# Chris10M/Lip2Speech

Hardware: AMD Instinct MI355X
Metric: mel-frames/sec at LRW batch=32, 29-frame clips (Lip2Speech.inference, S=300) (higher is better)
Workload: dtype f32; 1 GPU; LRW single-word, batch=32 per step, 29x96x96 RGB mouth crops, S=300 decode steps, speaker embedding supplied (encoding=voice), random-init weights; every step is one full pass over one B=32 batch; frames=29, decode_steps=300, library=libl2s_hip.so, parallelism=dp1 (clip sharding, no collective), batches_per_launch_chain=8, launch_chains_in_flight_per_gpu=3, distinct_batches_per_gpu=24, ranks=1

## Files before the change

### include/l2s_diag.h

```cpp
#ifndef L2S_DIAG_H
#define L2S_DIAG_H

#include "l2s.h"

#ifdef __cplusplus
extern "C" {
#endif


int l2s_op_gemm(const float* A, const float* Wt, const float* scale, const float* shift, const float* actw,
                float* C, int M, int N, int K, int act, void* stream);
int l2s_op_conv1d(const float* X, const float* Wp, const float* scale, const float* shift, const float* actw,
                  float* out, int B, int Tin, int Cin, int Cout, int taps, int stride, int pad, int act,
                  void* stream);
int l2s_op_gemm_ex(const float* A, const float* Wt, const float* scale, const float* shift, const float* actw, float* C, int M, int N,
                   int K, int act, int flags, void* stream);
int l2s_op_conv1d_ex(const float* X, const float* Wp, const float* scale, const float* shift, const float* actw, float* out, int B,
                     int Tin, int Cin, int Cout, int taps, int stride, int pad, int act, int flags, void* stream);
int l2s_op_conv1d_bwd(const float* dZ, const float* X, const float* Wp, float* dX, float* dWp, int B, int Tin, int Cin, int Cout, int taps,
                      int stride, int pad, void* stream);
int l2s_op_frontend(l2s_model* m, const float* video, int B, int T, int H, int W, float* out, void* stream);
int l2s_op_face_conv2d(const float* x, int64_t x_bstride, int B, int H, int W, int Cin, const float* w, const float* scale, const float* shift,
                       const float* res, int relu, float* y, int Cout, int kh, int kw, int stride, int ph, int pw, void* stream);
int l2s_op_face_taps(l2s_model* m, const float* faces, int64_t batch_stride, int B, float* const* taps, float* proj, float* emb, void* ws,
                     int64_t ws_bytes, void* stream);
int l2s_op_speaker_taps(l2s_model* m, const float* audio, int B, int n_samples, float* const* taps, float* emb, void* ws, int64_t ws_bytes, void* stream);
int l2s_op_speaker_taps_packed(l2s_model* m, const float* audio_packed, const int64_t* offsets, const int64_t* n_samples, int B, float* const* taps, float* emb,
                               void* ws, int64_t ws_bytes, void* stream);
int l2s_op_encoder_taps(l2s_model* m, const float* video, int B, int T, int H, int W, float* const* taps, float* feat, void* ws, int64_t ws_bytes,
                        void* stream);
int l2s_op_lstm_cell_chain(l2s_model* m, int B, int n_pairs, void* ws, int64_t ws_bytes, void* stream, double* avg_us);
int l2s_op_launch_chain(int kind, int n_launches, int blocks, int n_per_block, const float* in, float* out, void* stream);
int l2s_op_skinny_timeline(void* ts_dev);
int l2s_op_attn_timeline(void* ts_dev);
int l2s_op_flat_timeline(void* ts_dev);
int l2s_op_pdecode_timeline(void* ts_dev, int step);
int l2s_op_gemm_x3_timeline(void* ts_dev, int block);
int l2s_op_fused_unit_timeline(void* ts_dev, int h);
int l2s_op_step_attn_chain(l2s_model* m, float* state, int B, int T, int n_launches, void* ws, int64_t ws_bytes, void* stream);
int l2s_op_launch_chain2(int kind, int n_launches, int blocks, int n_per_block, const float* in, float* out, void* stream_a, void* stream_b);
int l2s_op_stamp_log(void* log_dev, int64_t capacity);

#ifdef __cplusplus
}
#endif
#endif
```

### lip2speech_amd/csrc/l2s_api.hip

```cpp
#include "../../include/l2s.h"
#ifdef L2S_DIAG
#include "../../include/l2s_diag.h"
#endif
#include "l2s_common.h"
#include "l2s_model.h"
#include "pdecode.h"

#include <algorithm>
#include <cmath>
#include <functional>
#include <cstring>
#include <map>
#include <memory>
#include <mutex>
#include <string>
#include <unordered_map>
#include <vector>

namespace l2s {

static thread_local std::string g_err;
void set_error(const std::string& msg) { g_err = msg; }

static Options g_default_opt;
// ... 56 lines not shown
void prof_count(const char* name, int64_t n) {
    if (!g_prof_on) return;
    std::lock_guard<std::mutex> lk(g_prof_mu);
    auto it = g_prof_idx.find(name);
    if (it == g_prof_idx.end()) {
        g_prof_idx[name] = (int)g_prof.size();
        g_prof.push_back(ProfEntry{name});
        it = g_prof_idx.find(name);
    }
    g_prof[it->second].launches += n;
}
static void prof_drain() {
    std::lock_guard<std::mutex> lk(g_prof_mu);
    for (auto& e : g_prof) {
        for (auto& pr : e.pending) {
            (void)hipEventSynchronize(pr.second);
            float ms = 0.f;
            if (hipEventElapsedTime(&ms, pr.first, pr.second) == hipSuccess) e.total_ms += ms;
            (void)hipEventDestroy(pr.first);
            (void)hipEventDestroy(pr.second);
        }
        e.pending.clear();
    }
}

}

namespace l2s {

struct EncPlan {
    int NF, Hp;
    int64_t act_a, act_b, t1, t2, last;
};
static EncPlan enc_plan(int NF, int H) {
    EncPlan p{};
    p.NF = NF;
    p.Hp = H / 4;
    int64_t hw = (int64_t)p.Hp * p.Hp;
    int64_t amax = (int64_t)p.NF * hw * STAGE_CH[0], t1 = 0, t2 = 0;
    int cin = STAGE_CH[0];
    int h = p.Hp;
    for (int st = 0; st < 3; ++st) {
        int cout = STAGE_CH[st + 1], half = cout / 2;
        int ho = (h + 1) / 2;
        int64_t in_px = (int64_t)p.NF * h * h, out_px = (int64_t)p.NF * ho * ho;
        t1 = std::max(t1, std::max(in_px * half, out_px * half));
        t2 = std::max(t2, std::max(out_px * cin, out_px * half));
        amax = std::max(amax, out_px * cout);
        cin = cout;
        h = ho;
    }
    p.act_a = amax; p.act_b = amax; p.t1 = t1; p.t2 = t2;
    p.last = (int64_t)p.NF * h * h * LAST_CH;
    return p;
}
static int64_t enc_ws_floats(int NF, int H) {
    EncPlan p = enc_plan(NF, H);
    return p.act_a + p.act_b + p.t1 + p.t2 + p.last + 64 * 8;
}

static int64_t prologue_ws_floats(int B, int T) {
    int L[4];
    int m = content_lens(T, L);
    int64_t BT = (int64_t)B * T, n = 0;
    n += BT * 4096;
    n += BT * 1024;
    n += BT * 512;
    n += (int64_t)B * 512 * 2;
    n += (int64_t)pad16(B) * 512 * 6;
    n += (int64_t)B * 1024;
    n += BT * 4608;
    for (int j = 0; j < 4; ++j) n += (int64_t)B * L[j] * 512;
    n += (int64_t)B * m * 2560;
    n += (int64_t)B * m * 256 * 4;
    n += (int64_t)B * m * (VOC + VOCP);
    n += 8 * std::max((int64_t)B * m * 256, (int64_t)B * 512);
    for (int j = 1; j < 4; ++j) n += (int64_t)CT_KS[j] * B * L[j] * 512;
    n += 8 * BT * 512;
    if (B <= 2) n += pbilstm_ws_bytes() / 4 + 64;
    return n + 64 * 44;
}
static int64_t decode_ws_floats(int B) {
    int64_t Bp = pad16(B);
    return Bp * (512 * 4 + 512 * 2 + 512 + 256 * 4 + 96) + (int64_t)B * (512 + 256 + 256) + 64 * 24 + (B + 2 + 64)  + (B <= 8 ? pdecode_ws_bytes(B) / 4 + 64 : 0);
}
constexpr int POST_TAPSPLIT_ROWS = 640;
static int64_t postnet_ws_floats(int B, int S) { return (int64_t)B * S * 512 * ((int64_t)B * S <= POST_TAPSPLIT_ROWS * MAX_GROUP ? 9 : 4) + 64 * 7; }


static GemmP pw_gemm(const float* A, int lda, int a_off, const ConvW& c, float* C, int ldc, int c_off, int cstride,
                     int64_t M, int N, int K, int act) {
    GemmP p = gemm_plain(A + a_off, lda, c.W, C + c_off, ldc, (int)M, N, K);
    p.scale = c.scale; p.shift = c.shift; p.actw = c.actw; p.act = act; p.c_cstride = cstride;
    p.W3 = c.W3;
    return p;
}

static FrameSrc frame_src(const float* video, int B) { FrameSrc f{}; f.p[0] = video; f.per = B; return f; }

#define S1_RUN_CHAINED(m, U, run, h) \
    ((m)->opt.trunk_chain && ((h) >= 6 || (m)->opt.trunk_chain >= 2) && (m)->opt.trunk_x3 && (U).pw1_p3 && (U).pw2_p3 && (run) >= 2 && (run) <= S1_CHAIN_MAX)
#ifdef L2S_DIAG
static int enc_tap(float* const* taps, int i, const float* src, int64_t n, hipStream_t s) {
    if (taps && taps[i]) L2S_CHECK_HIP(hipMemcpyAsync(taps[i], src, (size_t)n * sizeof(float), hipMemcpyDeviceToDevice, s));
    return 0;
}
static int enc_tap_interior(int u) {
    set_error("l2s: encoder tap of unit " + std::to_string(u) + " asked for, but the unit is interior to a stage-chain launch and its output never reaches memory (option \"trunk_chain\")");
    return 1;
}
static int enc_taps_check(const l2s_model* m, float* const* taps, int h) {
    if (!taps || !m->opt.fuse_trunk) return 0;
    for (int u = 0; u < N_UNITS; ++u) {
        const UnitW& U = m->w.unit[u];
        if (U.stride2) { h = (h + 1) / 2; continue; }
        int run = 1;
        while (u + run < N_UNITS && !m->w.unit[u + run].stride2 && m->w.unit[u + run].half == U.half) ++run;
        if (!S1_RUN_CHAINED(m, U, run, h)) continue;
        for (int i = 0; i < run - 1; ++i)
            if (taps[1 + u + i]) return enc_tap_interior(u + i);
        u += run - 1;
    }
    return 0;
}
#define L2S_ENC_TAP(i, src, n) do { if (enc_tap(taps, i, src, n, s)) return 1; } while (0)
#define L2S_ENC_TAPS_ARG , float* const* taps = nullptr
#else
#define L2S_ENC_TAP(i, src, n) do {} while (0)
#define L2S_ENC_TAPS_ARG
#endif
static int encoder_run(l2s_model* m, const FrameSrc& video, int B, int T, int H, int W, const float* emb, float* vis,
                       float* feat, void* ws, int64_t ws_bytes, hipStream_t s, const RaggedTab* rg = nullptr L2S_ENC_TAPS_ARG) {
    X3Scope x3scope(m->opt.infer_bf16 ? 0 : m->opt.gemm_x3);
    Bf16Scope bf16scope(m->opt.infer_bf16);
    const Weights& w = m->w;
    EncPlan pl = enc_plan(rg ? rg->NF : B * T, H);
    Bump bp(ws, ws_bytes);
    float* a = bp.f(pl.act_a); float* b = bp.f(pl.act_b); float* t1 = bp.f(pl.t1); float* t2 = bp.f(pl.t2); float* last = bp.f(pl.last);
    L2S_REQUIRE(!bp.overflow, "encoder workspace too small");
#ifdef L2S_DIAG
    if (enc_taps_check(m, taps, pl.Hp)) return 1;
#endif
    FrontendW fe = w.fe;
    if (!m->opt.frontend_x3) fe.w3 = nullptr;
    fe.pair = m->opt.frontend_x3 >= 2; fe.pipe = m->opt.frontend_x3 == 3;
    fe.solo = m->opt.frontend_solo && (m->opt.frontend_solo >= 2 || chains_hint() >= 2);
    if (!m->opt.infer_bf16) fe.w1 = nullptr;
    if (rg ? launch_frontend_ragged(fe, video, *rg, H, W, a, s) : launch_frontend(fe, video, B, T, H, W, a, s)) return 1;
    L2S_ENC_TAP(0, a, (int64_t)pl.NF * pl.Hp * pl.Hp * STAGE_CH[0]);
    float* x = a; float* y = b;
    int h = pl.Hp;
    const int NF = pl.NF;
    for (int u = 0; u < N_UNITS; ++u) {
        const UnitW& U = w.unit[u];
        const int half = U.half, cout = 2 * half;
        if (U.stride2 && m->opt.fuse_trunk && m->opt.fuse_s2) {
            ShuffleS2P sp{};
            sp.x = x; sp.out = y;
            sp.wd1 = U.b1_dw.w9; sp.sd1 = U.b1_dw.scale; sp.bd1 = U.b1_dw.shift;
            sp.wb1f = U.b1_frag; sp.sb1 = U.b1_pw.scale; sp.bb1 = U.b1_pw.shift;
            sp.w1f = U.pw1_frag; sp.s1 = U.pw1.scale; sp.b1 = U.pw1.shift;
            sp.wd = U.dw.w9; sp.sd = U.dw.scale; sp.bd = U.dw.shift;
            sp.w2f = U.pw2_frag; sp.s2 = U.pw2.scale; sp.b2 = U.pw2.shift;
            sp.NF = NF; sp.h = h; sp.ho = (h + 1) / 2; sp.cin = U.cin; sp.half = half; sp.Kin = U.kin; sp.Kh = U.kpad;
            sp.Ro = U.cin == 232 ? 3 : 2;
            if (m->opt.trunk_x3) { sp.wb1p = U.b1_p3; sp.w1p = U.pw1_p3; sp.w2p = U.pw2_p3; }
            if (launch_shuffle_s2(sp, s)) return 1;
// ... 206 lines not shown
        if (launch_gemm_splitk(p, 8, part, s, "prologue_gemm")) return 1;
        if (launch_stop_const(state + sl.ecell, w.stop_tail, w.stop_bias, B, state + sl.stopc, s)) return 1;
    }
    {
        GemmP p = gemm_plain(rnn, 1024, w.enc_proj.W, cat, 4608, BT, 512, 1024);
        p.shift = w.enc_proj.shift;
        p.R1 = resid; p.ldr1 = 512; p.r1_mod = 0;
        p.R2 = s_a; p.ldr2 = 512; p.r2_div = T;
        if (launch_gemm_splitk(p, 4, bott_part, s, "prologue_gemm")) return 1;
        if (lens ? launch_mask_copy_rows(cat, 4608, state + sl.enc, 512, lens.dev, B, T, 512, s)
                 : launch_copy_cols(cat, 4608, 0, state + sl.enc, 512, 0, 1, BT, 512, s)) return 1;
    }
    {
        GemmBatch gb{};
        int g = 0;
        for (int j = 3; j >= 0; --j)
            for (int kv = 0; kv < 2; ++kv)
                gb.p[g++] = conv_gemm(cat, 4608, B, T, 512, w.mh_branch[kv][j], 512, MH_KS[j], 1, MH_KS[j] / 2,
                                      cat + 512 + (kv * 4 + j) * 512, 4608, ACT_SILU);
        gb.count = 8;
        if (!m->opt.gemm_x3_dma) for (int i = 0; i < 8; ++i) gb.p[i].W3 = nullptr;
        if (launch_gemm(gb, s, "multihop_conv_gemm")) return 1;
        GemmBatch bb{};
        for (int kv = 0; kv < 2; ++kv) {
            GemmP p = gemm_plain(cat, 4608, w.mh_bott[kv].W, state + (kv == 0 ? sl.k : sl.v), 512, BT, 512, 2560);
            if (kv == 1) { p.a_split = 512; p.a_gap = 2048; }
            p.shift = w.mh_bott[kv].shift; p.act = ACT_PSINE; p.actw = w.mh_bott[kv].actw;
            p.R1 = w.pos; p.ldr1 = 512; p.r1_mod = T;
            bb.p[kv] = p;
        }
        bb.count = 2;
        if (launch_gemm_splitk_group(bb, 4, bott_part, s, "multihop_bottleneck_gemm")) return 1;
        if (w.vproj.W) {
            GemmP p = gemm_plain(state + sl.v, 512, w.vproj.W, state + sl.vp, 256, BT, 256, 512);
            p.shift = w.vproj.shift;
            if (launch_gemm1(p, s, "prologue_gemm")) return 1;
        }
    }
    {
        GemmBatch gb{};
        for (int j = 0; j < 4; ++j)
            gb.p[j] = conv_gemm(cat, 4608, B, T, 512, w.ct_branch[j], 512, CT_KS[j], CT_KS[j], 0, cmap[j], 512, ACT_SILU);
        gb.count = 4;
        if (launch_gemm_tapsplit(gb, tap_part, s, "content_agg_gemm")) return 1;
        PoolCatP pc{};
        pc.x[0] = cat; pc.L[0] = T; pc.ld[0] = 4608;
        for (int j = 0; j < 4; ++j) { pc.x[j + 1] = cmap[j]; pc.L[j + 1] = L[j]; pc.ld[j + 1] = 512; }
        pc.nmaps = 5; pc.B = B; pc.m = mT; pc.C = 512; pc.out = pooled;
        if (lens) {
            PoolDiv pd{};
            pd.div[0] = 1;
            for (int j = 0; j < 4; ++j) pd.div[j + 1] = CT_KS[j];
            if (launch_pool_cat_masked(pc, pd, lens.dev, s)) return 1;
        } else if (launch_pool_cat(pc, s)) return 1;
        const int R = B * mT;
        GemmP p = gemm_plain(pooled, 2560, w.ct_bott.W, wv, 256, R, 256, 2560);
        p.shift = w.ct_bott.shift;
        if (launch_gemm_splitk(p, 8, part, s, "content_gemm")) return 1;
        GemmBatch g1{};
        g1.p[0] = gemm_plain(wv, 256, w.ct_k0.W, tA, 256, R, 256, 256); g1.p[0].shift = w.ct_k0.shift; g1.p[0].act = ACT_SILU;
        g1.p[1] = gemm_plain(wv, 256, w.ct_fc0.W, tB, 256, R, 256, 256); g1.p[1].shift = w.ct_fc0.shift; g1.p[1].act = ACT_SILU;
        g1.count = 2;
        if (launch_gemm(g1, s, "content_gemm")) return 1;
        GemmBatch g2{};
        g2.p[0] = gemm_plain(tA, 256, w.ct_k2.W, state + sl.ckey, 256, R, 256, 256); g2.p[0].shift = w.ct_k2.shift; g2.p[0].act = ACT_SILU;
        g2.p[1] = gemm_plain(tB, 256, w.ct_fc2.W, tC, 256, R, 256, 256); g2.p[1].shift = w.ct_fc2.shift; g2.p[1].act = ACT_SILU;
        g2.count = 2;
        if (launch_gemm(g2, s, "content_gemm")) return 1;
        GemmP p3 = gemm_plain(tC, 256, w.ct_fc4.W, logits, VOC, R, VOC, 256);
        p3.shift = w.ct_fc4.shift; p3.act = ACT_SILU;
        if (launch_gemm1(p3, s, "content_gemm")) return 1;
        if (launch_gumbel_softmax(logits, gumbel, R, VOC, 0.1f, z, VOCP, content_dis, s)) return 1;
        if (lens && launch_zero_slot_rows(z, VOCP, content_dis, VOC, B, mT, lens.dev, s)) return 1;
        GemmP p4 = gemm_plain(z, VOCP, w.ct_emb.W, state + sl.cval, 256, R, 256, VOCP);
        if (launch_gemm1(p4, s, "content_gemm")) return 1;
    }
    if (launch_fill(state + sl.c, (int64_t)Bp * 512 * 2, 0.f, s)) return 1;
    return 0;
}


struct DecodeBufs {
    float *h0[2], *h1[2], *c0, *c1, *av, *p1, *cc, *uu, *yf, *p2f, *q, *qc, *p2;
};

static int decode_launches(l2s_model* m, float* state, int B, int T, int S, const float* teacher, const uint8_t* teacher_mask,
                           float* mel, float* stop, float* attn, int attn_logits, void* ws, int64_t ws_bytes, hipStream_t s, bool fold,
                           const std::function<int(int)>* on_frames = nullptr, bool early = false, ClipLens lens = {}) {
    const Weights& w = m->w;
    StateLayout sl = state_layout(B, T);
    const int Bp = pad16(B);
    const bool vhoist = fold && m->opt.hoist_vproj && w.lstm0v.W && w.vproj.W;
    const bool vsum = vhoist && m->opt.hoist_vproj >= 2 && skinny_sum_supported(m->opt);
    Bump bp(ws, ws_bytes);
    DecodeBufs d;
    for (int i = 0; i < 2; ++i) d.h0[i] = bp.f((int64_t)Bp * 512);
    for (int i = 0; i < 2; ++i) d.h1[i] = bp.f((int64_t)Bp * 512);
    d.c0 = bp.f((int64_t)Bp * 512); d.c1 = bp.f((int64_t)Bp * 512); d.av = bp.f((int64_t)Bp * 512);
    d.p1 = bp.f((int64_t)Bp * 256); d.cc = bp.f((int64_t)Bp * 256); d.uu = bp.f((int64_t)Bp * 256); d.p2f = bp.f((int64_t)Bp * 256);
    d.yf = bp.f((int64_t)Bp * 96);
    d.q = bp.f((int64_t)B * 512); d.qc = bp.f((int64_t)B * 256); d.p2 = bp.f((int64_t)B * 256);
    EsCtl* const es = early ? reinterpret_cast<EsCtl*>(bp.f(B + 2)) : nullptr;
    L2S_REQUIRE(!bp.overflow, "decode workspace too small");
    L2S_REQUIRE(!early || !teacher, "early stop is for free-running loops");
    if (es) L2S_CHECK_HIP(hipMemsetAsync(es, 0, sizeof(int) * (B + 2), s));
    const int* const es_end = es ? &es->end_rel : nullptr;

    L2S_CHECK_HIP(hipMemcpyAsync(d.h0[0], state + sl.h, sizeof(float) * Bp * 512, hipMemcpyDeviceToDevice, s));
    L2S_CHECK_HIP(hipMemcpyAsync(d.h1[0], state + sl.h + (int64_t)Bp * 512, sizeof(float) * Bp * 512, hipMemcpyDeviceToDevice, s));
    float* zero512[] = {d.h0[1], d.h1[1], d.c0, d.c1, d.av};
    for (float* z : zero512) if (launch_fill(z, (int64_t)Bp * 512, 0.f, s)) return 1;
    float* zero256[] = {d.p1, d.cc, d.uu, d.p2f};
    for (float* z : zero256) if (launch_fill(z, (int64_t)Bp * 256, 0.f, s)) return 1;
    if (launch_to_frag(w.bos, 0, B, 80, d.yf, 80, 0, 1, s)) return 1;

    auto fc_group = [&](int step, const float* h1buf, bool write_y) {
        SkinnyP a = sk_base(w.fc, B);
        a.seg[0] = {h1buf, 32}; a.nseg = 1; a.epi = SK_MEL;
        a.mel = mel + (int64_t)step * NM; a.ld_mel_b = (int64_t)S * NM;
        a.stop = stop + step; a.ld_stop_b = S; a.stop_const = state + sl.stopc; a.yfrag = write_y ? d.yf : nullptr;
        if (es) { a.es_ctl = reinterpret_cast<int*>(es); a.es_end = std::min(S, step + 1 + ES_MARGIN) - S; }
        return a;
    };

    for (int i = 0; i < S; ++i) {
        const int cur = i & 1, nxt = cur ^ 1;
        const bool forced = teacher && teacher_mask && teacher_mask[i];
        if (forced)
            if (launch_to_frag(teacher + (int64_t)i * NM, S * NM, B, 80, d.yf, 80, 0, 0, s)) return 1;
        {
            SkinnyBatch sb{};
            const bool from_frame = !fold || i == 0 || forced;
            SkinnyP a = sk_base(from_frame ? w.pre1 : w.pre1f, B);
            if (from_frame) a.seg[0] = {d.yf, 5}; else a.seg[0] = {d.h1[cur], 32};
            a.nseg = 1; a.act = ACT_PSINE; a.epi = SK_FRAG; a.out = d.p1; a.ldo = 256;
            SkinnyP b = sk_base(w.q, B);
            b.seg[0] = {d.h0[cur], 32}; b.seg[1] = {d.h1[cur], 32}; b.nseg = 2; b.act = ACT_PSINE; b.epi = SK_PLAIN; b.out = d.q; b.ldo = 512;
            b.addrow = w.pos + (int64_t)i * 512;
            SkinnyP c = sk_base(w.cq, B);
            c.seg[0] = {d.c0, 32}; c.seg[1] = {d.c1, 32}; c.nseg = 2; c.act = ACT_SILU; c.epi = SK_PLAIN; c.out = d.qc; c.ldo = 256;
            sb.p[0] = a; sb.ntiles[0] = 16;
            sb.p[1] = b; sb.ntiles[1] = w.q.tiles;
            sb.p[2] = c; sb.ntiles[2] = w.cq.tiles;
            sb.count = 3;
            if (fold && i > 0) { sb.p[3] = fc_group(i - 1, d.h1[cur], false); sb.ntiles[3] = w.fc.tiles; sb.count = 4; }
            sb.es_end = es_end; sb.es_step = (fold && i > 0 ? i - 1 : i) - S;
            if (launch_skinny(sb, s, fold ? "step_prenet1_q_cq_fc" : "step_prenet1_q_cq", m->opt)) return 1;
            if (fold && i > 0 && on_frames && (*on_frames)(i)) return 1;
        }
        {
            AttnP at{};
            at.q = d.q; at.ldq = 512; at.k = state + sl.k; at.v = state + sl.v; at.tau = w.tau; at.av_frag = d.av;
            if (fold && vhoist) at.vp = state + sl.vp;
            at.attn_out = attn ? attn + (int64_t)i * T : nullptr; at.ld_attn_b = (int64_t)S * T; at.attn_logits = attn_logits;
            at.qc = d.qc; at.ldqc = 256; at.ckey = state + sl.ckey; at.cval = state + sl.cval; at.tau_c = w.tau_c; at.cc_frag = d.cc;
            at.B = B; at.T = T; at.m = sl.m;
            at.es_end = es_end; at.es_step = i - S;
            SkinnyP pr = sk_base(w.pre2, B);
            pr.seg[0] = {d.p1, 16}; pr.nseg = 1; pr.act = ACT_PSINE;
            if (fold) { pr.epi = SK_FRAG; pr.out = d.p2f; pr.ldo = 256; }
            else { pr.epi = SK_PLAIN; pr.out = d.p2; pr.ldo = 256; }
            if (lens ? launch_step_attn_masked(at, pr, w.pre2.tiles, lens.dev, s, m->opt.attn_lds, m->opt.attn_skip0)
                     : launch_step_attn(at, pr, w.pre2.tiles, s, m->opt.attn_lds, m->opt.attn_skip0)) return 1;
        }
        if (!fold) {
            SkinnyBatch sb{};
            SkinnyP a = sk_base(w.aproj, B);
            a.seg[0] = {d.av, 32}; a.nseg = 1; a.epi = SK_FRAG; a.out = d.uu; a.ldo = 256; a.add = d.p2; a.ld_add = 256;
            sb.p[0] = a; sb.ntiles[0] = w.aproj.tiles; sb.count = 1;
            sb.es_end = es_end; sb.es_step = i - S;
            if (launch_skinny(sb, s, "step_attention_proj", m->opt)) return 1;
        }
        {
            SkinnyBatch sb{};
            SkinnyP a = sk_base(fold ? (vsum ? w.lstm0 : vhoist ? w.lstm0v : w.lstm0f) : w.lstm0, B);
            if (vsum) { a.seg[0] = {d.cc, 16}; a.seg[1] = {d.p2f, 16}; a.a_sum = d.av; a.seg[2] = {d.h0[cur], 32}; a.nseg = 3; }
            else if (fold) { a.seg[0] = {d.cc, 16}; a.seg[1] = {d.p2f, 16}; a.seg[2] = {d.av, vhoist ? 16 : 32}; a.seg[3] = {d.h0[cur], 32}; a.nseg = 4; }
            else { a.seg[0] = {d.cc, 16}; a.seg[1] = {d.uu, 16}; a.seg[2] = {d.h0[cur], 32}; a.nseg = 3; }
            a.epi = SK_LSTM; a.H = 512; a.c_in = d.c0; a.c_out = d.c0; a.h_out = d.h0[nxt]; a.h_out_K = 512; a.h_out_off = 0;
            sb.p[0] = a; sb.ntiles[0] = 128; sb.count = 1;
            sb.es_end = es_end; sb.es_step = i - S;
            if (launch_skinny(sb, s, "step_lstm_cell", m->opt)) return 1;
        }
        {
            SkinnyBatch sb{};
            SkinnyP a = sk_base(w.lstm1, B);
            a.seg[0] = {d.h0[nxt], 32}; a.seg[1] = {d.h1[cur], 32}; a.nseg = 2;
            a.epi = SK_LSTM; a.H = 512; a.c_in = d.c1; a.c_out = d.c1; a.h_out = d.h1[nxt]; a.h_out_K = 512; a.h_out_off = 0;
            sb.p[0] = a; sb.ntiles[0] = w.lstm1.tiles; sb.count = 1;
            sb.es_end = es_end; sb.es_step = i - S;
            if (launch_skinny(sb, s, "step_lstm_cell", m->opt)) return 1;
        }
        if (!fold || i == S - 1) {
            SkinnyBatch sb{};
            sb.p[0] = fc_group(i, d.h1[nxt], !fold); sb.ntiles[0] = w.fc.tiles; sb.count = 1;
            sb.es_end = es_end; sb.es_step = i - S;
            if (launch_skinny(sb, s, "step_fc_out_stop", m->opt)) return 1;
            if (on_frames && (*on_frames)(i + 1)) return 1;
        }
    }
    return 0;
}

static int side_stream_ready(l2s_model* m) {
    if (m->side) return 0;
    L2S_CHECK_HIP(hipStreamCreateWithFlags(&m->side, hipStreamNonBlocking));
    L2S_CHECK_HIP(hipEventCreateWithFlags(&m->ev_in, hipEventDisableTiming));
    L2S_CHECK_HIP(hipEventCreateWithFlags(&m->ev_out, hipEventDisableTiming));
    return 0;
}

static int decode_run(l2s_model* m, float* state, int B, int T, int S, const float* teacher, const uint8_t* teacher_mask,
                      float* mel, float* stop, float* attn, int attn_logits, void* ws, int64_t ws_bytes, hipStream_t s, bool may_stop_early, ClipLens lens = {}) {
    L2S_REQUIRE(S >= 1 && S <= L2S_MAX_STEPS, "S must be in [1, 300] (positional table)");
    const bool fold = m->opt.fold != 0 && m->folded_valid;
    const bool early = may_stop_early && m->opt.early_stop != 0 && !teacher;
    if (early) {
        L2S_CHECK_HIP(hipMemsetAsync(mel, 0, sizeof(float) * B * S * NM, s));
        L2S_CHECK_HIP(hipMemsetAsync(stop, 0, sizeof(float) * B * S, s));
        if (attn) L2S_CHECK_HIP(hipMemsetAsync(attn, 0, sizeof(float) * B * S * T, s));
    }
    const Weights& w = m->w;
    StateLayout sl = state_layout(B, T);
    const int pgate = (persist_envelope(m, (bool)lens, B, T, sl.m) && !teacher && fold && w.vproj.W && w.pre1f.W && w.lstm0.W && w.lstm1.W) ? pdecode_gate(T) : 0;
    if (pgate < 0) return 1;
    if (pgate > 0) {
        PDecP p{};
        p.Wq = w.q.W; p.bq = w.q.bias; p.aq = w.q.actw;
        p.Wcq = w.cq.W; p.bcq = w.cq.bias;
        p.Wp1f = w.pre1f.W; p.bp1f = w.pre1f.bias; p.ap1 = w.pre1f.actw;
        p.Wp1 = w.pre1.W; p.bp1 = w.pre1.bias;
        p.Wp2 = w.pre2.W; p.bp2 = w.pre2.bias; p.ap2 = w.pre2.actw;
        p.Wl0 = w.lstm0.W; p.bl0 = w.lstm0.bias; p.Wl1 = w.lstm1.W; p.bl1 = w.lstm1.bias;
        p.Wfc = w.fc.W; p.bfc = w.fc.bias;
        p.pos = w.pos; p.tau = w.tau; p.tau_c = w.tau_c; p.bos = w.bos;
        p.k = state + sl.k; p.vp = state + sl.vp; p.ckey = state + sl.ckey; p.cval = state + sl.cval;
        p.h_init = state + sl.h; p.stop_const = state + sl.stopc;
        p.mel = mel; p.stop = stop; p.attn = attn; p.attn_logits = attn_logits;
        p.B = B; p.T = T; p.m = sl.m; p.S = S;
        p.early = early ? ES_MARGIN : 0;
        return launch_pdecode(p, ws, ws_bytes, s, lens);
    }
    const bool use_graph = m->opt.graph && !teacher && !g_prof_on && !early && !lens;
    if (!use_graph) return decode_launches(m, state, B, T, S, teacher, teacher_mask, mel, stop, attn, attn_logits, ws, ws_bytes, s, fold, nullptr, early, lens);

    std::lock_guard<std::mutex> side_lock(m->side_mu);
    if (side_stream_ready(m)) return 1;
    l2s_model::GraphEntry* hit = nullptr;
    for (auto& g : m->graphs)
        if (g.B == B && g.T == T && g.S == S && g.attn_logits == attn_logits && g.fold == (int)fold && g.state == state && g.mel == mel &&
            g.stop == stop && g.attn == attn && g.ws == ws) { hit = &g; break; }
    if (!hit) {
        hipGraph_t graph = nullptr;
        L2S_CHECK_HIP(hipStreamBeginCapture(m->side, hipStreamCaptureModeThreadLocal));
        int rc = decode_launches(m, state, B, T, S, nullptr, nullptr, mel, stop, attn, attn_logits, ws, ws_bytes, m->side, fold);
        hipError_t ce = hipStreamEndCapture(m->side, &graph);
        if (rc) { if (graph) (void)hipGraphDestroy(graph); return 1; }
        L2S_CHECK_HIP(ce);
        hipGraphExec_t exec = nullptr;
        L2S_CHECK_HIP(hipGraphInstantiate(&exec, graph, nullptr, nullptr, 0));
        if (m->graphs.size() >= 8) {
            (void)hipGraphExecDestroy(m->graphs.front().exec);
            (void)hipGraphDestroy(m->graphs.front().graph);
            m->graphs.erase(m->graphs.begin());
        }
        m->graphs.push_back({B, T, S, attn_logits, (int)fold, state, mel, stop, attn, ws, graph, exec});
        hit = &m->graphs.back();
    }
    L2S_CHECK_HIP(hipEventRecord(m->ev_in, s));
    L2S_CHECK_HIP(hipStreamWaitEvent(m->side, m->ev_in, 0));
    L2S_CHECK_HIP(hipGraphLaunch(hit->exec, m->side));
    L2S_CHECK_HIP(hipEventRecord(m->ev_out, m->side));
    L2S_CHECK_HIP(hipStreamWaitEvent(s, m->ev_out, 0));
    return 0;
// ... 956 lines not shown
    if (!std::strcmp(name, "persist_decode") && value > 0) pdecode_rearm();
    return 0;
}

#ifdef L2S_DIAG
int l2s_op_lstm_cell_chain(l2s_model* m, int B, int n_pairs, void* ws, int64_t ws_bytes, void* stream, double* avg_us) {
    L2S_DEC_READY(m);
    L2S_REQUIRE(ws && avg_us && B > 0 && n_pairs > 0, "bad arguments");
    hipStream_t s = (hipStream_t)stream;
    const Weights& w = m->w;
    const int Bp = pad16(B);
    Bump bp(ws, ws_bytes);
    float* h0[2] = {bp.f((int64_t)Bp * 512), bp.f((int64_t)Bp * 512)};
    float* h1[2] = {bp.f((int64_t)Bp * 512), bp.f((int64_t)Bp * 512)};
    float* c0 = bp.f((int64_t)Bp * 512); float* c1 = bp.f((int64_t)Bp * 512); float* av = bp.f((int64_t)Bp * 512);
    float* cc = bp.f((int64_t)Bp * 256); float* p2f = bp.f((int64_t)Bp * 256);
    L2S_REQUIRE(!bp.overflow, "workspace too small");
    for (float* z : {h0[0], h0[1], h1[0], h1[1], c0, c1, av}) if (launch_fill(z, (int64_t)Bp * 512, 0.f, s)) return 1;
    for (float* z : {cc, p2f}) if (launch_fill(z, (int64_t)Bp * 256, 0.f, s)) return 1;
    hipEvent_t e0, e1;
    L2S_CHECK_HIP(hipEventCreate(&e0));
    L2S_CHECK_HIP(hipEventCreate(&e1));
    auto pair = [&](int cur) -> int {
        const int nxt = cur ^ 1;
        SkinnyBatch sb{};
        const bool vhoist = m->opt.hoist_vproj && w.lstm0v.W && w.vproj.W;
        const bool vsum = vhoist && m->opt.hoist_vproj >= 2 && skinny_sum_supported(m->opt);
        SkinnyP a = sk_base(vsum ? w.lstm0 : vhoist ? w.lstm0v : w.lstm0f, B);
        if (vsum) { a.seg[0] = {cc, 16}; a.seg[1] = {p2f, 16}; a.a_sum = av; a.seg[2] = {h0[cur], 32}; a.nseg = 3; }
        else { a.seg[0] = {cc, 16}; a.seg[1] = {p2f, 16}; a.seg[2] = {av, vhoist ? 16 : 32}; a.seg[3] = {h0[cur], 32}; a.nseg = 4; }
        a.epi = SK_LSTM; a.H = 512; a.c_in = c0; a.c_out = c0; a.h_out = h0[nxt]; a.h_out_K = 512; a.h_out_off = 0;
        sb.p[0] = a; sb.ntiles[0] = 128; sb.count = 1;
        if (launch_skinny(sb, s, "step_lstm_cell", m->opt)) return 1;
        SkinnyBatch sc{};
        SkinnyP b = sk_base(w.lstm1, B);
        b.seg[0] = {h0[nxt], 32}; b.seg[1] = {h1[cur], 32}; b.nseg = 2;
        b.epi = SK_LSTM; b.H = 512; b.c_in = c1; b.c_out = c1; b.h_out = h1[nxt]; b.h_out_K = 512; b.h_out_off = 0;
        sc.p[0] = b; sc.ntiles[0] = 128; sc.count = 1;
        return launch_skinny(sc, s, "step_lstm_cell", m->opt);
    };
    for (int i = 0; i < 8; ++i) if (pair(i & 1)) return 1;
    L2S_CHECK_HIP(hipEventRecord(e0, s));
    for (int i = 0; i < n_pairs; ++i) if (pair(i & 1)) return 1;
    L2S_CHECK_HIP(hipEventRecord(e1, s));
    L2S_CHECK_HIP(hipEventSynchronize(e1));
    float ms = 0.f;
    L2S_CHECK_HIP(hipEventElapsedTime(&ms, e0, e1));
    (void)hipEventDestroy(e0); (void)hipEventDestroy(e1);
    *avg_us = (double)ms * 1e3 / (2.0 * n_pairs);
    return 0;
}

int l2s_op_step_attn_chain(l2s_model* m, float* state, int B, int T, int n_launches, void* ws, int64_t ws_bytes, void* stream) {
    L2S_DEC_READY(m);
    L2S_REQUIRE(state && ws && B >= 1 && n_launches >= 1, "bad arguments");
    hipStream_t s = (hipStream_t)stream;
    const Weights& w = m->w;
    StateLayout sl = state_layout(B, T);
    const int Bp = pad16(B);
    Bump bp(ws, ws_bytes);
    float* q = bp.f((int64_t)B * 512); float* qc = bp.f((int64_t)B * 256);
    float* av = bp.f((int64_t)Bp * 512); float* cc = bp.f((int64_t)Bp * 256); float* p1 = bp.f((int64_t)Bp * 256); float* p2f = bp.f((int64_t)Bp * 256);
    L2S_REQUIRE(!bp.overflow, "workspace too small");
    if (launch_fill(q, (int64_t)B * 512, 0.f, s) || launch_fill(qc, (int64_t)B * 256, 0.f, s) || launch_fill(p1, (int64_t)Bp * 256, 0.f, s)) return 1;
    for (int i = 0; i < n_launches; ++i) {
        AttnP at{};
        at.q = q; at.ldq = 512; at.k = state + sl.k; at.v = state + sl.v; at.tau = w.tau; at.av_frag = av;
        if (m->opt.hoist_vproj && w.vproj.W) at.vp = state + sl.vp;
        at.attn_out = nullptr; at.ld_attn_b = 0; at.attn_logits = 0;
        at.qc = qc; at.ldqc = 256; at.ckey = state + sl.ckey; at.cval = state + sl.cval; at.tau_c = w.tau_c; at.cc_frag = cc;
        at.B = B; at.T = T; at.m = sl.m;
        SkinnyP pr = sk_base(w.pre2, B);
        pr.seg[0] = {p1, 16}; pr.nseg = 1; pr.act = ACT_PSINE; pr.epi = SK_FRAG; pr.out = p2f; pr.ldo = 256;
        if (launch_step_attn(at, pr, w.pre2.tiles, s, m->opt.attn_lds, m->opt.attn_skip0)) return 1;
    }
    return 0;
}
int l2s_op_skinny_timeline(void* ts_dev) { skinny_set_timeline((unsigned long long*)ts_dev); return 0; }
int l2s_op_attn_timeline(void* ts_dev) { attn_set_timeline((unsigned long long*)ts_dev); return 0; }
int l2s_op_flat_timeline(void* ts_dev) { skinny_set_flat_timeline((unsigned long long*)ts_dev); return 0; }
int l2s_op_pdecode_timeline(void* ts_dev, int step) { pdecode_set_timeline((unsigned long long*)ts_dev, step); return 0; }
int l2s_op_gemm_x3_timeline(void* ts_dev, int block) { gemm_x3_set_timeline((unsigned long long*)ts_dev, block); return 0; }
int l2s_op_fused_unit_timeline(void* ts_dev, int h) { shuffle_set_timeline((unsigned long long*)ts_dev, h); return 0; }
int l2s_op_stamp_log(void* log_dev, int64_t capacity) {
    L2S_REQUIRE(set_stamp_log((unsigned long long*)log_dev, (long long)capacity) == 0, "stamp log: hipMemcpyToSymbol failed");
    return 0;
}

int l2s_op_launch_chain(int kind, int n_launches, int blocks, int n_per_block, const float* in, float* out, void* stream) {
    for (int i = 0; i < n_launches; ++i)
        if (launch_probe(kind, blocks, n_per_block, in, out, (hipStream_t)stream)) return 1;
    return 0;
}

int l2s_op_launch_chain2(int kind, int n_launches, int blocks, int n_per_block, const float* in, float* out, void* stream_a, void* stream_b) {
    for (int i = 0; i < n_launches; ++i) {
        if (launch_probe(kind, blocks, n_per_block, in, out, (hipStream_t)stream_a)) return 1;
        if (launch_probe(kind, blocks, n_per_block, in + (int64_t)(1 << 24), out + 2048, (hipStream_t)stream_b)) return 1;
    }
    return 0;
}
#endif

int l2s_set_thread_chains(int n) { chains_hint() = n < 1 ? 1 : n; return 0; }
int l2s_persist_available(void) { return pdecode_device_ok() ? 1 : 0; }
int l2s_persist_timeouts(void) { return pdecode_timeouts(); }

int l2s_profile_enable(int on) { g_prof_on = on != 0; return 0; }
int l2s_profile_reset(void) { prof_drain(); g_prof.clear(); g_prof_idx.clear(); return 0; }
int l2s_profile_count(void) { prof_drain(); return (int)g_prof.size(); }
int l2s_profile_get(int idx, const char** name, int64_t* launches, double* total_ms) {
    prof_drain();
    L2S_REQUIRE(idx >= 0 && idx < (int)g_prof.size(), "profile index");
    if (name) *name = g_prof[idx].name.c_str();
    if (launches) *launches = g_prof[idx].launches;
    if (total_ms) *total_ms = g_prof[idx].total_ms;
    return 0;
}

}
```

### lip2speech_amd/csrc/l2s_common.h

```cpp
#pragma once
#include <hip/hip_runtime.h>
#include <stdint.h>
#include <string>

#define L2S_WAVE 64

typedef float f32x4 __attribute__((ext_vector_type(4)));
typedef float f32x16 __attribute__((ext_vector_type(16)));

namespace l2s {

void set_error(const std::string& msg);
#define L2S_CHECK_HIP(expr)                                                                   \
    do {                                                                                      \
        hipError_t _e = (expr);                                                               \
        if (_e != hipSuccess) {                                                               \
            l2s::set_error(std::string(#expr) + ": " + hipGetErrorString(_e));                \
            return 1;                                                                         \
        }                                                                                     \
    } while (0)
#define L2S_REQUIRE(cond, msg)                                                                \
    do {                                                                                      \
        if (!(cond)) {                                                                        \
            l2s::set_error(std::string("l2s: ") + (msg) + " [" #cond "]");                    \
// ... 154 lines not shown
                 const float* totals, int64_t rows, int C, hipStream_t s);
constexpr int DWS_RS = 1024;
int launch_dwconv_stats(const float* in, int N, int Hi, int Wi, int ldi, int ci_off, int C, int stride, const float* w9, float* partials, hipStream_t s,
                        float* raw_out = nullptr, int ldo = 0, int co_off = 0);
int launch_bn_apply(float* x, int64_t rows, int C, int ld, int co_off, const float* scale, const float* shift, hipStream_t s, bool fused = false);

struct FrontendW {
    const float* w;
    const float* scale;
    const float* shift;
    const float* slope;
    const float* w3;
    int pair = 0;
    int solo = 0;
    int pipe = 0;
    const float* w1;
};
constexpr int MAX_GROUP = 8;
struct FrameSrc { const float* p[MAX_GROUP]; int per; };
int launch_frontend(const FrontendW& w, const FrameSrc& video, int B, int T, int H, int W, float* out, hipStream_t s, float* zout = nullptr);
inline int launch_frontend(const FrontendW& w, const float* video, int B, int T, int H, int W, float* out, hipStream_t s, float* zout = nullptr) {
    FrameSrc f{}; f.p[0] = video; f.per = B;
    return launch_frontend(w, f, B, T, H, W, out, s, zout);
}
struct RaggedClip { int g, row, T, len, frame0, pair0; };
constexpr int RAGGED_CHUNK = 32;
struct RaggedChunk { RaggedClip c[RAGGED_CHUNK]; int n; };
struct RaggedTab { const RaggedClip* clips; const int* pair_clip; int N, Tmax, NF, NP; };
int launch_ragged_table(const RaggedClip* clips_host, int N, RaggedClip* clips_dev, int* pair_clip_dev, hipStream_t s);
int launch_frontend_ragged(const FrontendW& w, const FrameSrc& video, const RaggedTab& rg, int H, int W, float* out, hipStream_t s);
struct EvalClip { int S, T, row, mT, mel_off, stop_off, attn_off, dis_off; };
constexpr int EVAL_CHUNK = 32;
struct EvalChunk { EvalClip c[EVAL_CHUNK]; int n; };
struct EvalTab { const EvalClip* clips; int N, Smax, Tmax, mTmax; };
enum EvalField { EV_STOP = 0, EV_ATTN = 1, EV_DIS = 2, EV_MEL_POST = 3 };
int launch_eval_table(const EvalClip* clips_host, int N, EvalClip* clips_dev, hipStream_t s);
int launch_zero_rows_past_s(float* x, int cols, const EvalTab& ev, hipStream_t s);
int launch_eval_scatter(int field, const float* src, const EvalTab& ev, float* dst, hipStream_t s);
int launch_eval_mel_cf(const float* mel, const EvalTab& ev, float* mel_cf, hipStream_t s);
int launch_frontend_stats(const FrontendW& w, const float* video, int B, int T, int H, int W, float* partials , int* nblocks, hipStream_t s, float* raw_out = nullptr);
int launch_frontend_pool(const float* z, const float* slope, int NF, int Hc, int Wc, float* out, hipStream_t s);

constexpr int MAX_COLLATE_CLIPS = 64;
int launch_normalise_pad(const uint8_t* packed, const int64_t* offsets, const int* frames, int B, int T, int H, int W, float* video, hipStream_t s);
int launch_dwconv(const float* in, int N, int Hi, int Wi, int ldi, int ci_off, int C, int stride,
                  const float* w9 , const float* scale, const float* shift,
                  float* out, int ldo, int co_off, hipStream_t s);
struct ShuffleS1P {
    const float* x; float* out;
    const float* w1f; const float* s1; const float* b1;
    const float* wd; const float* sd; const float* bd;
    const float* w2f; const float* s2; const float* b2;
    int NF, h, half, Kpad, F;
    const void* w1p; const void* w2p;
};
int64_t su_planes_bytes(int N, int K);
int launch_su_planes(const float* W, int N, int K, void* out, hipStream_t s);
int launch_shuffle_s1(const ShuffleS1P& p, hipStream_t s);
constexpr int S1_CHAIN_MAX = 7;
int launch_shuffle_s1_chain(const ShuffleS1P* units, int n, hipStream_t s);
void shuffle_set_timeline(unsigned long long* ts, int h);
struct ShuffleS2P {
    const float* x; float* out;
    const float* wd1; const float* sd1; const float* bd1;
    const float* wb1f; const float* sb1; const float* bb1;
    const float* w1f; const float* s1; const float* b1;
    const float* wd; const float* sd; const float* bd;
    const float* w2f; const float* s2; const float* b2;
    int NF, h, ho, cin, half, Kin, Kh, Ro;
    const void* wb1p; const void* w1p; const void* w2p;
};
int launch_shuffle_s2(const ShuffleS2P& p, hipStream_t s);
int launch_copy_cols(const float* in, int ldi, int off_i, float* out, int ldo, int off_o, int cs_o,
                     int64_t rows, int cols, hipStream_t s);
int launch_pool_norm_cat(const float* x, int NF, int P, int C, const float* emb, int E, int T,
                         float* vis, int ldv, float* feat , hipStream_t s);
int launch_pool_norm_cat_ragged(const float* x, const RaggedTab& rg, int P, int C, const float* emb, int E, float* vis, int ldv, hipStream_t s);

__host__ __device__ inline int64_t frag16_index(int row, int k, int K) {
    int rt = row >> 4, i = row & 15, c = k >> 4, g = (k >> 2) & 3, e = k & 3;
    return ((int64_t)(rt * (K >> 4) + c) * 64 + (g * 16 + i)) * 4 + e;
}

enum SkinnyEpi {
    SK_PLAIN = 0,
    SK_FRAG = 1,
    SK_LSTM = 2,
    SK_MEL = 3,
};
struct SkinnySeg { const float* a; int nchunks; };
struct SkinnyP {
    SkinnySeg seg[4];
    int nseg;
    const float* a_sum;
    int layout;
    const float* W;
    const void* W3;
    const float* bias;
    const float* actw;
    const float* add;
    int ld_add;
    const float* addrow;
    float* out;
    int ldo;
    int B, N, K;
    int act;
    int epi;
    const float* pre;
    int64_t ld_pre;
    const float* c_in;
    float* c_out;
    float* h_out;
    int h_out_K, h_out_off;
    float* h_seq;
    int64_t ld_hseq;
    float* h_plain;
    int ld_hplain;
    int H;
    float* mel; int64_t ld_mel_b;
    float* stop; int64_t ld_stop_b;
    const float* stop_const;
    float* yfrag;
    int* es_ctl; int es_end;
};
struct EsCtl { int end_rel; int count; int crossed[1]; };
constexpr int ES_POST_LAYERS = 5, ES_POST_TAPS = 5;
constexpr int ES_MARGIN = ES_POST_LAYERS * (ES_POST_TAPS / 2);
constexpr int SKINNY_MAX_GROUP = 4;
struct SkinnyBatch { SkinnyP p[SKINNY_MAX_GROUP]; int ntiles[SKINNY_MAX_GROUP]; int count; const int* es_end; int es_step; };
#define L2S_ES_RETURN(arg) do { if ((arg).es_end && (arg).es_step >= *(arg).es_end) return; } while (0)
int launch_skinny(const SkinnyBatch& b, hipStream_t s, const char* name, const Options& o = Options());
int launch_skx_planes(const float* Wf, int ntiles, int K, void* out, hipStream_t s);
bool skinny_sum_supported(const Options& o);
void attn_set_timeline(unsigned long long* ts);
void skinny_set_flat_timeline(unsigned long long* ts);
void skinny_set_timeline(unsigned long long* ts);

int launch_probe(int kind, int blocks, int n_per_block, const float* in, float* out, hipStream_t s);
void skinny_set_flat_timeline(unsigned long long* ts);
int set_stamp_log(unsigned long long* log, long long cap);

struct AttnP {
    const float* q; int ldq;
    const float* k;
    const float* v;
    const float* vp;
    const float* tau;
    float* av_frag;
    float* attn_out; int64_t ld_attn_b; int attn_logits;
    const float* qc; int ldqc;
    const float* ckey;
    const float* cval;
    const float* tau_c;
    float* cc_frag;
    int B, T, m;
    const int* es_end; int es_step;
};
int launch_step_attn(const AttnP& at, const SkinnyP& pre2, int pre2_tiles, hipStream_t s, int lds_values = 1, int skip0 = 0);
struct PoolCatP { const float* x[5]; int L[5]; int ld[5]; int nmaps; int B, m, C; float* out; };
int launch_pool_cat(const PoolCatP& p, hipStream_t s);
int launch_gumbel_softmax(const float* logits, const float* gumbel, int rows, int n, float tau,
                          float* z, int ldz, float* dis, hipStream_t s);
int launch_to_frag(const float* x, int ldx, int B, int K, float* frag, int Kfrag, int koff, int broadcast_row, hipStream_t s);
int launch_fill(float* p, int64_t n, float v, hipStream_t s);
int launch_from_frag(const float* frag, int Kfrag, int B, int K, float* out, int ldo, int ooff, hipStream_t s);
int launch_tile_rows(const float* src, int lds, float* dst, int ldd, int B, int T, int C, hipStream_t s);
int launch_transpose_bsc(const float* in, int B, int S, int C, float* out, hipStream_t s);
int launch_output_lengths(const float* stop, int B, int S, int64_t* lengths, hipStream_t s);
int launch_mask_by_lengths(const int64_t* lengths, int B, int S, int T, float* mel_post, float* attn, hipStream_t s);
constexpr int LEN_CHUNK = 64;
struct LenChunk { int len[LEN_CHUNK]; int n; };
int launch_len_table(const int32_t* lens_host, int B, int* table, hipStream_t s);
int launch_bilstm_capture(const float* h_frag, const float* c_frag, const int* lens, int B, int t, float* h_dst_frag, float* c_dst, int ld_c, hipStream_t s);
int launch_bilstm_reset(float* h_frag, float* c_frag, const int* lens, int B, int t, const float* s_e, hipStream_t s);
int launch_mask_copy_rows(float* x, int ldx, float* out, int ldo, const int* lens, int B, int T, int cols, hipStream_t s);
struct PoolDiv { int div[5]; };
int launch_pool_cat_masked(const PoolCatP& p, const PoolDiv& d, const int* lens, hipStream_t s);
int launch_zero_slot_rows(float* z, int ldz, float* dis, int n, int B, int m, const int* lens, hipStream_t s);
int launch_step_attn_masked(const AttnP& at, const SkinnyP& pre2, int pre2_tiles, const int* lens, hipStream_t s, int lds_values = 1, int skip0 = 0);
int launch_frame_window(const float* audio, int B, int N, int L, int n_fft, int hop, const float* window, float* frames, hipStream_t s);
int launch_power(const float* spec, int lds, int64_t rows, int nf, float* power, int ldp, hipStream_t s);
struct SpkRank { int64_t off; int32_t n; int32_t b; };
constexpr int SPK_CHUNK = 512;
struct SpkChunk { int32_t v[SPK_CHUNK]; int n; };
int launch_spk_table(const int32_t* words_host, int64_t n_words, int32_t* table, hipStream_t s);
int launch_frame_window_packed(const float* audio_packed, const SpkRank* ranks, const int* step_row0, int B, int L_max, int n_fft, int hop, const float* window,
                               float* frames, hipStream_t s);
int launch_spk_last_hidden(const float* hseq, const SpkRank* ranks, const int* step_row0, int B, float* h_last, hipStream_t s);
constexpr int IM_MAXF = 576;
constexpr int IM_MAXM = 128;
constexpr int IM_NNZ = 2048;
int launch_mel_bands(const float* fb, int n_freqs, int n_mels, int* tab, float* fwd, float* bwd, hipStream_t s);
int launch_stop_const(const float* ecell, const float* w_tail, const float* bias, int B, float* out, hipStream_t s);

}
```

### lip2speech_amd/csrc/skinny.hip

```cpp
#include "l2s_common.h"
#include "skinny_dev.h"

#include <algorithm>

namespace l2s {

#ifdef L2S_DIAG
__device__ unsigned long long* d_stamp_log = nullptr;
__device__ unsigned long long d_stamp_cap = 0;
struct BlockStamp {
    unsigned long long t0 = 0;
    unsigned long long* log = nullptr;
    __device__ __forceinline__ void begin() { log = d_stamp_log; if (log && threadIdx.x == 0) t0 = wall_clock64(); }
    __device__ __forceinline__ void end(unsigned kind, const void* key) {
        if (!log) return;
        __syncthreads();
        if (threadIdx.x == 0) {
            const unsigned long long t1 = wall_clock64();
            const unsigned long long slot = atomicAdd(log, 1ull);
            if (slot < d_stamp_cap) {
                unsigned long long* r = log + 1 + 3 * slot;
                r[0] = t0; r[1] = t1; r[2] = ((unsigned long long)kind << 60) | ((unsigned long long)(uintptr_t)key & 0xFFFFFFFFFFFFull);
            }
        }
// ... 39 lines not shown
    const int lay = p.layout;
    if (MAXC == 12 && lay == 3) skinny_block<false, 12, false, SegLay<16, 16, 32, 32>>(p, blockIdx.x, blockIdx.y, red, batch.ntiles[g]);
    else if (MAXC >= 8 && lay == 2) skinny_block<false, 8, false, SegLay<32, 32, 0, 0>>(p, blockIdx.x, blockIdx.y, red, batch.ntiles[g]);
    else if (MAXC >= 4 && lay == 1) skinny_block<false, 4, false, SegLay<32, 0, 0, 0>>(p, blockIdx.x, blockIdx.y, red, batch.ntiles[g]);
    else if (lay == 4) skinny_block<false, 2, false, SegLay<16, 0, 0, 0>>(p, blockIdx.x, blockIdx.y, red, batch.ntiles[g]);
    else skinny_block<false, MAXC>(p, blockIdx.x, blockIdx.y, red, batch.ntiles[g]);
}
template <int MAXC, int NB, int WPS, bool ES = false>
__global__ __launch_bounds__(512, WPS) void skinny_kernel_split(const SkinnyBatch batch) {
    if constexpr (ES) L2S_ES_RETURN(batch);
    __shared__ float red[SK_RED_FLOATS];
    const int g = blockIdx.z;
    skinny_block<false, MAXC, false, SegRuntime, NB>(batch.p[g], blockIdx.x, blockIdx.y, red, batch.ntiles[g]);
}

template <int RT, int CT, int MAXC, int JB, int WPS, int DEPTH = 2, bool ES = false>
__global__ __launch_bounds__(512, WPS) void skinny_rc_kernel(const SkinnyBatch batch, int mts) {
    if constexpr (ES) L2S_ES_RETURN(batch);
    __shared__ float red[SkRc<RT, CT>::RED_FLOATS];
    const int g = blockIdx.z;
    skinny_block_rc<RT, CT, MAXC, JB, DEPTH>(batch.p[g], blockIdx.x, blockIdx.y, red, batch.ntiles[g], mts);
}
template <int LAYID> struct SkLay;
template <> struct SkLay<1> { using T = SegLay<32, 0, 0, 0>; };
template <> struct SkLay<2> { using T = SegLay<32, 32, 0, 0>; };
template <> struct SkLay<3> { using T = SegLay<16, 16, 32, 32>; };
template <> struct SkLay<5> { using T = SegLay<16, 16, 16, 32>; };
template <> struct SkLay<6> { using T = SegLay<16, 16, 32, 0, true>; };
template <int RT, int CT, int LAYID, int DEPTH, int WPS, bool IS_LSTM, bool ES = false>
__global__ __launch_bounds__(512, WPS) void skinny_rcs_kernel(const SkinnyBatch batch, int mts) {
    if constexpr (ES) L2S_ES_RETURN(batch);
    __shared__ float red[SkRc<RT, CT>::RED_FLOATS];
    const int g = blockIdx.z;
    skinny_block_rcs<RT, CT, typename SkLay<LAYID>::T, DEPTH, IS_LSTM>(batch.p[g], blockIdx.x, blockIdx.y, red, batch.ntiles[g], mts);
}
template <int RT, int CT, int LAYID, int DEPTH, bool IS_LSTM, bool ES = false>
__global__ __launch_bounds__(256, 1) void skinny_rc4_kernel(const SkinnyBatch batch, int mts) {
    if constexpr (ES) L2S_ES_RETURN(batch);
    __shared__ float red[SkRc<RT, CT>::RED_FLOATS];
    const int g = blockIdx.z;
    skinny_block_rcs<RT, CT, typename SkLay<LAYID>::T, DEPTH, IS_LSTM, false, 4>(batch.p[g], blockIdx.x, blockIdx.y, red, batch.ntiles[g], mts);
}
template <int RT, int CT, int LAYID, int DEPTH, bool ES = false>
__global__ __launch_bounds__(256, 1) void skinny_rc4x_kernel(const SkinnyBatch batch, int mts) {
    if constexpr (ES) L2S_ES_RETURN(batch);
    __shared__ float red[SkRc<RT, CT>::RED_FLOATS];
    const int g = blockIdx.z;
    skinny_block_rcs<RT, CT, typename SkLay<LAYID>::T, DEPTH, true, false, 4, true>(batch.p[g], blockIdx.x, blockIdx.y, red, batch.ntiles[g], mts);
}
template <int RT, int CT, int LAYID, int DEPTH, bool ES = false>
__global__ __launch_bounds__(256, 2) void skinny_rc4h_kernel(const SkinnyBatch batch, int mts) {
    if constexpr (ES) L2S_ES_RETURN(batch);
    __shared__ float red[SkRc<RT, CT>::RED_FLOATS];
    const int g = blockIdx.z;
    L2S_BLOCK_STAMP_BEGIN();
    skinny_block_rcs<RT, CT, typename SkLay<LAYID>::T, DEPTH, true, false, 4, true, false, true>(batch.p[g], blockIdx.x, blockIdx.y, red, batch.ntiles[g], mts);
    L2S_BLOCK_STAMP_END(1u, batch.p[g].c_out);
}
template <int RT, int CT, int LAYID, int DEPTH, bool ES = false>
__global__ __launch_bounds__(512, 1) void skinny_rc8x_kernel(const SkinnyBatch batch, int mts) {
    if constexpr (ES) L2S_ES_RETURN(batch);
    __shared__ float red[SkRc<RT, CT>::RED_FLOATS];
    const int g = blockIdx.z;
    L2S_BLOCK_STAMP_BEGIN();
    skinny_block_rcs<RT, CT, typename SkLay<LAYID>::T, DEPTH, true, false, 8, true>(batch.p[g], blockIdx.x, blockIdx.y, red, batch.ntiles[g], mts);
    L2S_BLOCK_STAMP_END(1u, batch.p[g].c_out);
}
template <int LAYID, bool ES = false>
__global__ __launch_bounds__(512, 1) void skinny_sp_kernel(const SkinnyBatch batch, int mts) {
    if constexpr (ES) L2S_ES_RETURN(batch);
    extern __shared__ __attribute__((aligned(16))) float sp_lds[];
    const int g = blockIdx.z;
    L2S_BLOCK_STAMP_BEGIN();
    skinny_block_sp<typename SkLay<LAYID>::T>(batch.p[g], blockIdx.x, blockIdx.y, sp_lds, batch.ntiles[g], mts);
    L2S_BLOCK_STAMP_END(4u, batch.p[g].c_out);
}
template <int LAYID>
static int launch_sp(const SkinnyBatch& bl, int maxt, int mts, hipStream_t s) {
    static const hipError_t attr = hipFuncSetAttribute(reinterpret_cast<const void*>(skinny_sp_kernel<LAYID, false>), hipFuncAttributeMaxDynamicSharedMemorySize, SKP_LDS_BYTES);
    L2S_CHECK_HIP(attr);
    static const hipError_t attr_es = hipFuncSetAttribute(reinterpret_cast<const void*>(skinny_sp_kernel<LAYID, true>), hipFuncAttributeMaxDynamicSharedMemorySize, SKP_LDS_BYTES);
    L2S_CHECK_HIP(attr_es);
    SK_ES_LAUNCH(bl.es_end, skinny_sp_kernel, (LAYID), dim3(maxt / 4, (mts + 3) / 4, bl.count), dim3(512), SKP_LDS_BYTES, s, bl, mts);
    L2S_CHECK_HIP(hipGetLastError());
    return 0;
}
__global__ __launch_bounds__(256) void skx_planes_kernel(const float4* __restrict__ Wf, int ntiles, int NC, uint4* __restrict__ out) {
    const int NPI = NC / 16;
    const int64_t total = (int64_t)ntiles * 8 * NPI * 64;
    for (int64_t i = (int64_t)blockIdx.x * 256 + threadIdx.x; i < total; i += (int64_t)gridDim.x * 256) {
        const int lane = (int)(i & 63);
        int64_t r = i >> 6;
        const int ip = (int)(r % NPI); r /= NPI;
        const int sl = (int)(r & 7);
        const int64_t tile = r >> 3;
        const float4 f0 = Wf[(tile * NC + sl + 16 * ip) * 64 + lane], f1 = Wf[(tile * NC + sl + 16 * ip + 8) * 64 + lane];
        uint2 h0, m0, l0, h1, m1, l1;
        skx_split4(f0, h0, m0, l0); skx_split4(f1, h1, m1, l1);
        uint4* o = out + (((tile * 8 + sl) * NPI + ip) * 3) * 64 + lane;
        o[0] = make_uint4(h0.x, h0.y, h1.x, h1.y); o[64] = make_uint4(m0.x, m0.y, m1.x, m1.y); o[128] = make_uint4(l0.x, l0.y, l1.x, l1.y);
    }
}
int launch_skx_planes(const float* Wf, int ntiles, int K, void* out, hipStream_t s) {
    L2S_REQUIRE(Wf && out && K % 256 == 0, "split-bf16 LSTM planes: K must be a multiple of 256 (whole chunk pairs per slice)");
    const int64_t total = (int64_t)ntiles * 8 * (K / 256) * 64;
    hipLaunchKernelGGL(skx_planes_kernel, dim3((unsigned)std::min<int64_t>((total + 255) / 256, 4096)), dim3(256), 0, s, reinterpret_cast<const float4*>(Wf), ntiles, K / 16,
                       reinterpret_cast<uint4*>(out));
    L2S_CHECK_HIP(hipGetLastError());
    return 0;
}

template <int RT, int CT, int DEPTH>
static bool launch_rc4(const SkinnyBatch& bl, int lay, int kind, int maxt, int mts, hipStream_t s, int x3 = 0) {
    const dim3 grid((maxt + CT - 1) / CT, (mts + RT - 1) / RT, bl.count), blk(256);
    constexpr int HD = 3;
    if constexpr (RT * CT >= 8) {
        if (kind == 2 && x3 == 3 && (lay == 1 || lay == 2 || lay == 6)) {
            if (lay == 1) SK_ES_LAUNCH(bl.es_end, skinny_rc4h_kernel, (RT, CT, 1, HD), grid, blk, 0, s, bl, mts);
            else if (lay == 2) SK_ES_LAUNCH(bl.es_end, skinny_rc4h_kernel, (RT, CT, 2, HD), grid, blk, 0, s, bl, mts);
            else SK_ES_LAUNCH(bl.es_end, skinny_rc4h_kernel, (RT, CT, 6, HD), grid, blk, 0, s, bl, mts);
            return true;
        }
    }
    if (kind == 2 && x3 >= 2 && (lay == 1 || lay == 2 || lay == 6)) {
        if (lay == 1) SK_ES_LAUNCH(bl.es_end, skinny_rc8x_kernel, (RT, CT, 1, DEPTH), grid, dim3(512), 0, s, bl, mts);
        else if (lay == 2) SK_ES_LAUNCH(bl.es_end, skinny_rc8x_kernel, (RT, CT, 2, DEPTH), grid, dim3(512), 0, s, bl, mts);
        else SK_ES_LAUNCH(bl.es_end, skinny_rc8x_kernel, (RT, CT, 6, DEPTH), grid, dim3(512), 0, s, bl, mts);
        return true;
    }
    if (kind == 2 && x3 && (lay == 1 || lay == 2 || lay == 6)) {
        if (lay == 1) SK_ES_LAUNCH(bl.es_end, skinny_rc4x_kernel, (RT, CT, 1, DEPTH), grid, blk, 0, s, bl, mts);
        else if (lay == 2) SK_ES_LAUNCH(bl.es_end, skinny_rc4x_kernel, (RT, CT, 2, DEPTH), grid, blk, 0, s, bl, mts);
        else SK_ES_LAUNCH(bl.es_end, skinny_rc4x_kernel, (RT, CT, 6, DEPTH), grid, blk, 0, s, bl, mts);
        return true;
    }
    if (kind == 2) {
        if (lay == 1) SK_ES_LAUNCH(bl.es_end, skinny_rc4_kernel, (RT, CT, 1, DEPTH, true), grid, blk, 0, s, bl, mts);
        else if (lay == 2) SK_ES_LAUNCH(bl.es_end, skinny_rc4_kernel, (RT, CT, 2, DEPTH, true), grid, blk, 0, s, bl, mts);
        else if (lay == 3) SK_ES_LAUNCH(bl.es_end, skinny_rc4_kernel, (RT, CT, 3, DEPTH, true), grid, blk, 0, s, bl, mts);
        else if (lay == 5) SK_ES_LAUNCH(bl.es_end, skinny_rc4_kernel, (RT, CT, 5, DEPTH, true), grid, blk, 0, s, bl, mts);
        else if (lay == 6) SK_ES_LAUNCH(bl.es_end, skinny_rc4_kernel, (RT, CT, 6, DEPTH, true), grid, blk, 0, s, bl, mts);
        else return false;
    } else if (kind == 1) {
        if (lay == 1) SK_ES_LAUNCH(bl.es_end, skinny_rc4_kernel, (RT, CT, 1, DEPTH, false), grid, blk, 0, s, bl, mts);
        else if (lay == 2) SK_ES_LAUNCH(bl.es_end, skinny_rc4_kernel, (RT, CT, 2, DEPTH, false), grid, blk, 0, s, bl, mts);
        else return false;
    } else return false;
    return true;
}
#ifdef L2S_DIAG
template <int LAYID, bool X3 = false, int NW = 4>
__global__ __launch_bounds__(64 * NW, 1) void skinny_rcs_timed_kernel(const SkinnyBatch batch, int mts, unsigned long long* ts) {
    __shared__ float red[SkRc<4, 2>::RED_FLOATS];
    const int blk = blockIdx.y * gridDim.x + blockIdx.x;
    skinny_block_rcs<4, 2, typename SkLay<LAYID>::T, 4, true, true, NW, X3>(batch.p[0], blockIdx.x, blockIdx.y, red, batch.ntiles[0], mts, ts + (int64_t)blk * 8);
}
#endif
template <int RT, int CT, int DEPTH>
static bool launch_rcs(const SkinnyBatch& bl, int lay, int kind, int maxt, int mts, hipStream_t s) {
    const dim3 grid((maxt + CT - 1) / CT, (mts + RT - 1) / RT, bl.count), blk(512);
    if (kind == 2) {
        if (lay == 1) SK_ES_LAUNCH(bl.es_end, skinny_rcs_kernel, (RT, CT, 1, DEPTH, 2, true), grid, blk, 0, s, bl, mts);
        else if (lay == 2) SK_ES_LAUNCH(bl.es_end, skinny_rcs_kernel, (RT, CT, 2, DEPTH, 2, true), grid, blk, 0, s, bl, mts);
        else if (lay == 3) SK_ES_LAUNCH(bl.es_end, skinny_rcs_kernel, (RT, CT, 3, DEPTH, 2, true), grid, blk, 0, s, bl, mts);
        else if (lay == 5) SK_ES_LAUNCH(bl.es_end, skinny_rcs_kernel, (RT, CT, 5, DEPTH, 2, true), grid, blk, 0, s, bl, mts);
        else return false;
// ... 73 lines not shown
        if (fl.wide[k]) skinny_block_rcs<R8, C8, SegLay<32, 32, 0, 0>, 8, false, TIMED>(p, tp, mg, red, batch.ntiles[g], mts, tb);
        else skinny_block_rcs<R4, C4, SegLay<32, 0, 0, 0>, 4, false, TIMED>(p, tp, mg, red, batch.ntiles[g], mts, tb);
    } else {
        if (fl.wide[k]) skinny_block_rc<R8, C8, 8, 2>(p, tp, mg, red, batch.ntiles[g], mts);
        else skinny_block_rc<R4, C4, 4, 2>(p, tp, mg, red, batch.ntiles[g], mts);
    }
    L2S_BLOCK_STAMP_END(2u, batch.p[0].out);
}
static int plan_flat(const SkinnyBatch& bl, int mts, int cap, SkinnyFlat& fl, bool half = false, bool xcd = false) {
    static const int S8[2] = {21, 22}, S4[3] = {21, 22, 42};
    const int n = bl.count;
    auto shape_of = [&](int g, int s8, int s4) { return bl.p[g].K > 512 ? s8 : s4; };
    auto nblocks = [&](int g, int sh) { return ((bl.ntiles[g] + sh % 10 - 1) / (sh % 10)) * ((mts + sh / 10 - 1) / (sh / 10)); };
    auto nbytes = [&](int g, int sh) { return (int64_t)(16 * (sh / 10) + 16 * (sh % 10)) * bl.p[g].K * 4; };
    auto cost = [&](int g, int sh) { return (double)nbytes(g, sh) / 36.5e3 + 2.0 * 256 * (sh / 10) * (sh % 10) * bl.p[g].K / 350e3; };
    int best8 = 0, best4 = 0;
    double best_max = -1;
    int64_t best_sum = 0;
    for (int s8 : S8)
        for (int s4 : S4) {
            if (half && s4 == 42) continue;
            int blocks = 0; double mx = 0; int64_t sum = 0;
            for (int g = 0; g < n; ++g) {
                const int sh = shape_of(g, s8, s4);
                blocks += nblocks(g, sh); mx = std::max(mx, cost(g, sh)); sum += nbytes(g, sh) * nblocks(g, sh);
            }
            if (blocks <= cap && (best_max < 0 || mx < best_max - 1e-9 || (mx < best_max + 1e-9 && sum < best_sum))) { best_max = mx; best_sum = sum; best8 = s8; best4 = s4; }
        }
    if (best_max < 0) return 0;
    int order[SKINNY_MAX_GROUP] = {0, 1, 2, 3};
    std::stable_sort(order, order + n, [&](int a, int b) { return nbytes(a, shape_of(a, best8, best4)) > nbytes(b, shape_of(b, best8, best4)); });
    int pos = 0;
    for (int k = 0; k < n; ++k) {
        const int g = order[k], sh = shape_of(g, best8, best4);
        fl.first[k] = pos; fl.gid[k] = g;
        fl.ncol[k] = (bl.ntiles[g] + sh % 10 - 1) / (sh % 10);
        fl.wide[k] = bl.p[g].K > 512 ? 1 : 0;
        fl.nrow[k] = (mts + sh / 10 - 1) / (sh / 10);
        fl.xcd[k] = (xcd && pos % 8 == 0 && fl.nrow[k] % 2 == 0 && fl.ncol[k] % 4 == 0) ? 1 : 0;
        pos += nblocks(g, sh);
    }
    for (int k = n; k <= SKINNY_MAX_GROUP; ++k) fl.first[k] = pos;
    return best8 * 100 + best4;
}
#ifdef L2S_DIAG
static unsigned long long* g_flat_ts = nullptr;
void skinny_set_flat_timeline(unsigned long long* ts) { g_flat_ts = ts; }
#endif
template <int S8, int S4>
static void launch_flat(const SkinnyBatch& bl, const SkinnyFlat& fl, int mts, hipStream_t s, int stat) {
#ifdef L2S_DIAG
    if (g_flat_ts && stat == 1) {
        if constexpr (S8 == 22 && S4 == 42) { hipLaunchKernelGGL((skinny_flat_kernel<S8, S4, 1, true>), dim3(fl.first[SKINNY_MAX_GROUP]), dim3(512), 0, s, bl, fl, mts, g_flat_ts); return; }
    }
#endif
    if (stat == 2) SK_ES_LAUNCH(bl.es_end, skinny_flat_kernel, (S8, S4, 2, false), dim3(fl.first[SKINNY_MAX_GROUP]), dim3(256), 0, s, bl, fl, mts, (unsigned long long*)nullptr);
    else if (stat == 1) SK_ES_LAUNCH(bl.es_end, skinny_flat_kernel, (S8, S4, 1, false), dim3(fl.first[SKINNY_MAX_GROUP]), dim3(512), 0, s, bl, fl, mts, (unsigned long long*)nullptr);
    else SK_ES_LAUNCH(bl.es_end, skinny_flat_kernel, (S8, S4, 0, false), dim3(fl.first[SKINNY_MAX_GROUP]), dim3(512), 0, s, bl, fl, mts, (unsigned long long*)nullptr);
}

#ifdef L2S_DIAG
__global__ __launch_bounds__(512) void skinny_kernel_timed(const SkinnyBatch batch, unsigned long long* ts) {
    __shared__ float red[SK_RED_FLOATS];
    const int g = blockIdx.z;
    const int blk = (blockIdx.z * gridDim.y + blockIdx.y) * gridDim.x + blockIdx.x;
    const SkinnyP& p = batch.p[g];
    if (p.layout == 3) skinny_block<false, 12, true, SegLay<16, 16, 32, 32>>(p, blockIdx.x, blockIdx.y, red, batch.ntiles[g], nullptr, ts + (int64_t)blk * 8);
    else if (p.layout == 2) skinny_block<false, 8, true, SegLay<32, 32, 0, 0>>(p, blockIdx.x, blockIdx.y, red, batch.ntiles[g], nullptr, ts + (int64_t)blk * 8);
    else skinny_block<false, SK_MAXC, true>(p, blockIdx.x, blockIdx.y, red, batch.ntiles[g], nullptr, ts + (int64_t)blk * 8);
}
#endif
#ifdef L2S_DIAG
static unsigned long long* g_skinny_ts = nullptr;
#else
static constexpr unsigned long long* g_skinny_ts = nullptr;
#endif
#ifdef L2S_DIAG
void skinny_set_timeline(unsigned long long* ts) { g_skinny_ts = ts; }
#endif

static bool skinny_shape_known(int shape) { return shape == 0 || shape == 11 || shape == 21 || shape == 22 || shape == 42; }
bool skinny_sum_supported(const Options& o) { return o.rc_jb == 0 && g_skinny_ts == nullptr && skinny_shape_known(o.rc_shape) && skinny_shape_known(o.rc_shape_multi); }

int launch_skinny(const SkinnyBatch& b, hipStream_t s, const char* name, const Options& o) {
    L2S_REQUIRE(b.count >= 1 && b.count <= SKINNY_MAX_GROUP, "skinny group size");
    int maxt = 0, mts = 0;
    for (int i = 0; i < b.count; ++i) {
        const SkinnyP& p = b.p[i];
        int k = 0;
        for (int j = 0; j < 4; ++j) k += 16 * p.seg[j].nchunks;
        L2S_REQUIRE(k == p.K && p.K % 16 == 0 && p.K <= 16 * SK_WAVES * SK_MAXC, "skinny K segments");
        L2S_REQUIRE(p.B >= 1, "skinny B");
        maxt = b.ntiles[i] > maxt ? b.ntiles[i] : maxt;
        int m = (p.B + 15) / 16;
        L2S_REQUIRE(mts == 0 || mts == m, "skinny groups must share B");
        mts = m;
    }
    SkinnyBatch bl = b;
    for (int i = 0; i < bl.count; ++i) {
        for (int j = bl.p[i].nseg; j < 4; ++j) { bl.p[i].seg[j].nchunks = 0; bl.p[i].seg[j].a = bl.p[i].seg[0].a; }
        bl.p[i].layout = o.skinny_static ? skinny_layout_of(bl.p[i]) : 0;
    }
    ProfScope ps(name, s);
    int maxk = 0;
    for (int i = 0; i < bl.count; ++i) maxk = bl.p[i].K > maxk ? bl.p[i].K : maxk;
    const int cls = !o.skinny_sized ? 12 : maxk <= 512 ? 4 : maxk <= 1024 ? 8 : 12;
    int shape = (bl.count > 1 && o.rc_shape_multi) ? o.rc_shape_multi : o.rc_shape;
    bool n_lstm_all = o.rc_jb == 0;
    for (int i = 0; i < bl.count; ++i) n_lstm_all = n_lstm_all && bl.p[i].epi == SK_LSTM && bl.p[i].W3;
    if (shape == 0) {
        shape = 11;
        if (mts >= 4) {
            auto blocks = [&](int rt, int ct) { int n = 0; for (int i = 0; i < bl.count; ++i) n += (bl.ntiles[i] + ct - 1) / ct; return n * ((mts + rt - 1) / rt); };
            if (blocks(4, 2) >= 224 || (o.lstm_x3 >= 3 && chains_hint() >= 2 && o.half_min_mts > 0 && mts >= o.half_min_mts && n_lstm_all)) shape = 42;
            else if (blocks(2, 2) >= 224) shape = 22;
            else if (blocks(2, 1) >= 224) shape = 21;
        }
    }
    int rc_lay = skinny_layout_of(bl.p[0]);
    for (int i = 1; i < bl.count; ++i) if (skinny_layout_of(bl.p[i]) != rc_lay) rc_lay = 0;
    if (rc_lay == 4) rc_lay = 0;
    int n_lstm = 0;
    for (int i = 0; i < bl.count; ++i) n_lstm += bl.p[i].epi == SK_LSTM ? 1 : 0;
    const int rc_kind = n_lstm == bl.count ? 2 : n_lstm == 0 ? 1 : 0;
    const bool overlap = chains_hint() >= 2;
    int x3 = (o.rc_jb == 0 && rc_kind == 2 && (rc_lay == 1 || rc_lay == 2 || rc_lay == 6)) ? o.lstm_x3 : 0;
    if (x3 >= 3 && !overlap) x3 = 2;
    for (int i = 0; i < bl.count; ++i) if (!bl.p[i].W3) x3 = 0;
    if (x3 == 4) {
        bool sp = shape == 42 && !g_skinny_ts && o.half_min_mts > 0 && mts >= o.half_min_mts && (rc_lay == 2 || rc_lay == 6);
        for (int i = 0; i < bl.count; ++i) sp = sp && bl.ntiles[i] > 0 && bl.ntiles[i] % 4 == 0;
        if (sp) return rc_lay == 2 ? launch_sp<2>(bl, maxt, mts, s) : launch_sp<6>(bl, maxt, mts, s);
        x3 = 3;
    }
    if (!g_skinny_ts && bl.count > 1 && mts >= 8 && o.skinny_flat && !o.rc_shape && !o.rc_shape_multi && maxk <= 1024 && rc_kind == 1) {
        SkinnyFlat fl{};
        const bool half = o.flat_half != 0 && (o.flat_half >= 2 || chains_hint() >= 2);
        const int plan = plan_flat(bl, mts, half ? 512 : 256, fl, half, o.flat_xcd != 0);
        int stat = half ? 2 : o.rc_jb == 0 || o.rc_jb == 28 ? 1 : o.rc_jb == 44 ? 2 : 0;
        for (int i = 0; i < bl.count; ++i) if (!(skinny_layout_of(bl.p[i]) == (bl.p[i].K > 512 ? 2 : 1) && bl.p[i].epi != SK_LSTM)) stat = 0;
        if (plan) {
            switch (plan) {
                case 2121: launch_flat<21, 21>(bl, fl, mts, s, stat); break;
                case 2122: launch_flat<21, 22>(bl, fl, mts, s, stat); break;
                case 2142: launch_flat<21, 42>(bl, fl, mts, s, stat); break;
                case 2221: launch_flat<22, 21>(bl, fl, mts, s, stat); break;
                case 2222: launch_flat<22, 22>(bl, fl, mts, s, stat); break;
                default: launch_flat<22, 42>(bl, fl, mts, s, stat); break;
            }
            L2S_CHECK_HIP(hipGetLastError());
            return 0;
        }
    }
    for (int i = 0; i < bl.count; ++i)
        L2S_REQUIRE(!bl.p[i].a_sum || (rc_lay == 6 && rc_kind == 2 && skinny_sum_supported(o) && skinny_shape_known(shape) && shape != 0),
                    "skinny: a summed segment needs the straight-line LSTM blocks (shape 11 / 21 / 22 / 42, default operand batching)");
    bool any_sum = false;
    for (int i = 0; i < bl.count; ++i) any_sum = any_sum || bl.p[i].a_sum;
#ifdef L2S_DIAG
    if (g_skinny_ts && shape == 42 && bl.count == 1 && rc_kind == 2 && (rc_lay == 2 || rc_lay == 3)) {
        const dim3 grid((maxt + 1) / 2, (mts + 3) / 4, 1);
        if (rc_lay == 3) hipLaunchKernelGGL(skinny_rcs_timed_kernel<3>, grid, dim3(256), 0, s, bl, mts, g_skinny_ts);
        else if (x3 == 2) hipLaunchKernelGGL((skinny_rcs_timed_kernel<2, true, 8>), grid, dim3(512), 0, s, bl, mts, g_skinny_ts);
        else if (x3) hipLaunchKernelGGL((skinny_rcs_timed_kernel<2, true>), grid, dim3(256), 0, s, bl, mts, g_skinny_ts);
        else hipLaunchKernelGGL(skinny_rcs_timed_kernel<2>, grid, dim3(256), 0, s, bl, mts, g_skinny_ts);
    }
    else if (g_skinny_ts) hipLaunchKernelGGL(skinny_kernel_timed, dim3(maxt, mts, b.count), dim3(512), 0, s, bl, g_skinny_ts);
    else
#endif
    if (shape == 11 && o.rc_jb == 0 && rc_lay && rc_kind && launch_rc4<1, 1, 4>(bl, rc_lay, rc_kind, maxt, mts, s, x3)) {}
    else if (shape == 42) launch_rc<4, 2>(bl, cls, maxt, mts, s, o.rc_jb, rc_lay, rc_kind, x3);
    else if (shape == 22) launch_rc<2, 2>(bl, cls, maxt, mts, s, o.rc_jb, rc_lay, rc_kind, x3);
    else if (shape == 21) launch_rc<2, 1>(bl, cls, maxt, mts, s, o.rc_jb, rc_lay, rc_kind, x3);
    else if (any_sum) L2S_REQUIRE(false, "skinny: no block form of this launch sums u = prenet + o in its loader (SkinnyP::a_sum would be ignored)");
    else if (cls == 4) SK_ES_LAUNCH(bl.es_end, skinny_kernel, (4), dim3(maxt, mts, b.count), dim3(512), 0, s, bl);
    else if (cls == 8 && o.skinny_split8 == 2) SK_ES_LAUNCH(bl.es_end, skinny_kernel_split, (8, 2, 8), dim3(maxt, mts, b.count), dim3(512), 0, s, bl);
    else if (cls == 8) SK_ES_LAUNCH(bl.es_end, skinny_kernel, (8), dim3(maxt, mts, b.count), dim3(512), 0, s, bl);
    else if (cls == 12 && o.skinny_split == 2) SK_ES_LAUNCH(bl.es_end, skinny_kernel_split, (12, 2, 6), dim3(maxt, mts, b.count), dim3(512), 0, s, bl);
    else if (cls == 12 && o.skinny_split == 3) SK_ES_LAUNCH(bl.es_end, skinny_kernel_split, (12, 3, 8), dim3(maxt, mts, b.count), dim3(512), 0, s, bl);
    else SK_ES_LAUNCH(bl.es_end, skinny_kernel, (12), dim3(maxt, mts, b.count), dim3(512), 0, s, bl);
    L2S_CHECK_HIP(hipGetLastError());
    return 0;
}

struct StepB {
    AttnP at;
    SkinnyP pre2;
    int pre2_tiles;
    int mts;
};

constexpr int ATT_PRE2_MAXC = 2;
template <bool VL, bool SKIP0 = false, bool ES = false>
__global__ __launch_bounds__(512) void step_attn_kernel(const StepB sb) {
    constexpr int SMF = ATT_SM_FLOATS + (VL && !SKIP0 ? ATT_VLDS_FLOATS : 0);
    __shared__ __attribute__((aligned(16))) float sm[SMF > SK_RED_FLOATS ? SMF : SK_RED_FLOATS];
    if constexpr (ES) L2S_ES_RETURN(sb.at);
    const int nb = sb.at.B, ptiles = sb.pre2_tiles;
    L2S_PIN_S("s"(nb), "s"(ptiles));
    const int bid = blockIdx.x;
    L2S_BLOCK_STAMP_BEGIN();
    if (bid < nb) {
        attention_block<false, false, VL, SKIP0>(sb.at, bid, sm);
    } else if (bid < 2 * nb) {
        content_block(sb.at, bid - nb, sm);
    } else {
        const int j = bid - 2 * nb;
        const int tile = j % ptiles, mt = j / ptiles;
        skinny_block<false, ATT_PRE2_MAXC>(sb.pre2, tile, mt, sm);
    }
    L2S_BLOCK_STAMP_END(3u, sb.at.q);
}
// ... 112 lines not shown
```

### lip2speech_amd/csrc/skinny_dev.h

```cpp
#pragma once
#include "l2s_common.h"

#include <type_traits>
#include <utility>

namespace l2s {

struct SkinnyTrain {
    float* zsave; int ld_z;
    float* gates; int64_t ld_gates;
    float* c_new; int64_t ld_c;
    float* out_plain; int ld_out;
    const float* out_mask; int ld_mask;
    float* h_drop; int h_drop_K; const float* h_mask; int ld_hmask;
    const float* lb_gates; const float* lb_cprev; const float* lb_cnew; float* lb_dc; const float* lb_dha; int lb_ld_a; const float* lb_mask;
    float* lb_frag; float* lb_stack; int lb_H; int lb_ld_dc;
    float* lb_stack2; int64_t lb_ld_stack2;
    const float* add_hi; int add_hi_from;
    const float* sd_z; const float* sd_w; const float* sd_mask; float* sd_stack; float* sd_frag_d; float* sd_frag_dz; int sd_lo, sd_hi;
    float* sd_stack_dz;
};
struct AttnTrain {
    const float* logit_mask; int ld_lmask;
    float* alpha; int ld_alpha;
// ... 372 lines not shown
            __builtin_amdgcn_sched_barrier(0);
#pragma unroll
            for (int j = (bt + PRE) * JB; j < (bt + PRE + 1) * JB; ++j) load_chunk(j);
            __builtin_amdgcn_sched_barrier(0);
        }
    }
    {
        const int col = lane & 15, rb = 4 * (lane >> 4);
#pragma unroll
        for (int q = 0; q < NT; ++q)
#pragma unroll
            for (int r = 0; r < 4; ++r) red[((wave * NT + q) * 16 + rb + r) * 17 + col] = acc[q][0][r] + acc[q][1][r];
    }
    __syncthreads();
    float* gt = red + SK_WAVES * NT * 16 * 17;
#pragma unroll
    for (int n = 0; n < NQ; ++n) {
        const int q = half + 2 * n;
        if (q >= NT) continue;
        const int t = tp * CT + q % CT, rt = mg * RT + q / CT;
        if (t >= ntiles || rt >= mts) continue;
        float v = 0.f;
#pragma unroll
        for (int wv = 0; wv < SK_WAVES; ++wv) v += red[((wv * NT + q) * 16 + e_row) * 17 + e_col];
        v += pf_bias[n];
        const int b = rt * 16 + e_row, np = t * 16 + e_col;
        if (epi == SK_LSTM) {
            v += pf_extra[n];
            gt[(q * 16 + e_row) * 17 + e_col] = v;
            continue;
        }
        if (b >= nB) continue;
        if (epi == SK_MEL) {
            if (np < 80) {
                p.mel[(int64_t)b * p.ld_mel_b + np] = v;
                if (p.yfrag) p.yfrag[frag16_index(b, np, 80)] = v;
            } else if (np == 80) {
                p.stop[(int64_t)b * p.ld_stop_b] = v + p.stop_const[b];
                sk_note_stop(p, b, v + p.stop_const[b]);
            }
            continue;
        }
        if (np >= N) continue;
        v = act_apply(v, act, p.actw, np);
        v += pf_extra[n];
        if (epi == SK_FRAG) p.out[frag16_index(b, np, p.ldo)] = v;
        else p.out[(int64_t)b * p.ldo + np] = v;
    }
    if (epi != SK_LSTM) return;
    __syncthreads();
#pragma unroll
    for (int cr = 0; cr < NCR; ++cr) {
        if (!cell_on[cr]) continue;
        const int q2 = (tid >> 6) + 8 * cr;
        const int t2 = tp * CT + q2 % CT, rt2 = mg * RT + q2 / CT;
        const int b2 = rt2 * 16 + (t64 >> 2), unit2 = t2 * 4 + (t64 & 3);
        const int r2 = t64 >> 2, u2 = t64 & 3;
        const float* g4 = gt + (q2 * 16 + r2) * 17 + 4 * u2;
        const float gi = g4[0], gf = g4[1], gg = g4[2], go = g4[3];
        const float cn = sigmoidf_(gf) * pf_c[cr] + sigmoidf_(gi) * tanhf(gg);
        const float hn = sigmoidf_(go) * tanhf(cn);
        p.c_out[frag16_index(b2, unit2, H)] = cn;
        p.h_out[frag16_index(b2, p.h_out_off + unit2, p.h_out_K)] = hn;
        if (p.h_seq) p.h_seq[(int64_t)b2 * p.ld_hseq + unit2] = hn;
        if (p.h_plain) p.h_plain[(int64_t)b2 * p.ld_hplain + unit2] = hn;
    }
}

typedef __bf16 skx_bf16x8 __attribute__((ext_vector_type(8)));
__device__ __forceinline__ void skx_split4(const float4& v, uint2& hi, uint2& mid, uint2& lo) {
    const float f[4] = {v.x, v.y, v.z, v.w};
    unsigned h[4], m[4], l[4];
#pragma unroll
    for (int e = 0; e < 4; ++e) {
        const unsigned xb = __float_as_uint(f[e]);
        const float r1 = f[e] - __uint_as_float(xb & 0xFFFF0000u);
        const float r2 = r1 - __uint_as_float(__float_as_uint(r1) & 0xFFFF0000u);
        h[e] = xb; m[e] = __float_as_uint(r1); l[e] = __float_as_uint(r2);
    }
    hi = make_uint2(__builtin_amdgcn_perm(h[1], h[0], 0x07060302u), __builtin_amdgcn_perm(h[3], h[2], 0x07060302u));
    mid = make_uint2(__builtin_amdgcn_perm(m[1], m[0], 0x07060302u), __builtin_amdgcn_perm(m[3], m[2], 0x07060302u));
    lo = make_uint2(__builtin_amdgcn_perm(l[1], l[0], 0x07060302u), __builtin_amdgcn_perm(l[3], l[2], 0x07060302u));
}
__device__ __forceinline__ void skx_split8(const float4& a, const float4& b, skx_bf16x8& hi, skx_bf16x8& mid, skx_bf16x8& lo) {
    uint2 h0, m0, l0, h1, m1, l1;
    skx_split4(a, h0, m0, l0); skx_split4(b, h1, m1, l1);
    hi = __builtin_bit_cast(skx_bf16x8, make_uint4(h0.x, h0.y, h1.x, h1.y));
    mid = __builtin_bit_cast(skx_bf16x8, make_uint4(m0.x, m0.y, m1.x, m1.y));
    lo = __builtin_bit_cast(skx_bf16x8, make_uint4(l0.x, l0.y, l1.x, l1.y));
}

__device__ __forceinline__ int sk_red_idx(int slot, int row, int col) { return slot * 256 + ((row ^ ((row >> 2) & 1)) << 4) + (col ^ ((row >> 1) & 3)); }
template <int RT, int CT, class LAY, int DEPTH, bool IS_LSTM, bool TIMED = false, int NW = SK_WAVES, bool X3 = false, bool TRAIN = false, bool SEQ = false>
__device__ __forceinline__ void skinny_block_rcs(const SkinnyP& p, int tp, int mg, float* red, int ntiles, int mts, unsigned long long* ts = nullptr,
                                                 const SkinnyTrain* tr = nullptr) {
    static_assert(!TRAIN || IS_LSTM, "the training stores of this form: the LSTM cell's tape (gates, new cell, dropped-out hidden state)");
    static_assert(NW == 8 || NW == 4, "eight waves, or four that each play two");
    static_assert(!X3 || (IS_LSTM && (LAY::NC / SK_WAVES) % 2 == 0), "the split-bf16 form: LSTM blocks, whole chunk pairs per slice");
    static_assert(!SEQ || NW == 4, "slices one after the other: the four-wave form");
    constexpr int VW = SK_WAVES / NW, NH = NW / 4;
    constexpr int VA = SEQ ? 1 : VW;
    L2S_STAMP(0);
    static_assert(LAY::STATIC && LAY::NC % SK_WAVES == 0, "static layout, every wave the same number of chunks");
    constexpr int NT = RT * CT, MAXC = LAY::NC / SK_WAVES, TC = MAXC * VW, NQ = (NT + NH - 1) / NH, PRE = TC < DEPTH ? TC : DEPTH, NC = LAY::NC;
    constexpr int E0 = LAY::n0, E1 = E0 + LAY::n1, E2 = E1 + LAY::n2;
    const float* const W = p.W;
    const float* const sa0 = p.seg[0].a; const float* const sa1 = p.seg[1].a; const float* const sa2 = p.seg[2].a; const float* const sa3 = p.seg[3].a;
    L2S_PIN_S("s"(W), "s"(sa0), "s"(sa1), "s"(sa2), "s"(sa3), "s"(ntiles), "s"(mts));
    if (tp * CT >= ntiles) return;
    L2S_STAMP(1);
    const int tid = threadIdx.x, lane = tid & 63;
    const int wave = __builtin_amdgcn_readfirstlane(tid >> 6);

    const __amdgpu_buffer_rsrc_t rs_w = __builtin_amdgcn_make_buffer_rsrc(const_cast<float*>(W), 0, 0x7fffffff, 0x00020000);
    const __amdgpu_buffer_rsrc_t rs_a0 = __builtin_amdgcn_make_buffer_rsrc(const_cast<float*>(sa0), 0, 0x7fffffff, 0x00020000);
    const __amdgpu_buffer_rsrc_t rs_a1 = __builtin_amdgcn_make_buffer_rsrc(const_cast<float*>(sa1), 0, 0x7fffffff, 0x00020000);
    const __amdgpu_buffer_rsrc_t rs_a2 = __builtin_amdgcn_make_buffer_rsrc(const_cast<float*>(sa2), 0, 0x7fffffff, 0x00020000);
    const __amdgpu_buffer_rsrc_t rs_a3 = __builtin_amdgcn_make_buffer_rsrc(const_cast<float*>(sa3), 0, 0x7fffffff, 0x00020000);
    int wo[CT];
#pragma unroll
    for (int i = 0; i < CT; ++i) wo[i] = ((min(tp * CT + i, ntiles - 1) * NC + wave) * 64 + lane) * 16;
    int ao[4][RT];
#pragma unroll
    for (int r = 0; r < RT; ++r) {
        const int rt = min(mg * RT + r, mts - 1);
        ao[0][r] = ((rt * LAY::n0 + wave) * 64 + lane) * 16;
        ao[1][r] = ((rt * LAY::n1 + wave) * 64 + lane) * 16;
        ao[2][r] = ((rt * LAY::n2 + wave) * 64 + lane) * 16;
        ao[3][r] = ((rt * LAY::n3 + wave) * 64 + lane) * 16;
    }
    constexpr int NS1 = LAY::SUM1 ? (LAY::n1 / SK_WAVES) * VW : 1;
    constexpr int FS1 = (E0 / SK_WAVES) * VW;
    const __amdgpu_buffer_rsrc_t rs_s1 = __builtin_amdgcn_make_buffer_rsrc(const_cast<float*>(LAY::SUM1 ? p.a_sum : W), 0, 0x7fffffff, 0x00020000);
    constexpr int NPI = MAXC / 2;
    const __amdgpu_buffer_rsrc_t rs_w3 = __builtin_amdgcn_make_buffer_rsrc(const_cast<void*>(X3 ? p.W3 : (const void*)W), 0, 0x7fffffff, 0x00020000);
    int wo3[CT];
#pragma unroll
    for (int i = 0; i < CT; ++i) wo3[i] = (((min(tp * CT + i, ntiles - 1) * SK_WAVES + wave) * NPI * 3) * 64 + lane) * 16;
    float4 a[TC][RT], w[X3 ? 1 : TC][CT], a2[NS1][RT];
    uint4 w3[X3 ? TC / 2 : 1][CT][3];
    auto load_chunk = [&](auto jc) {
        constexpr int t_ = decltype(jc)::value, j = t_;
        constexpr int jj_ = SEQ ? t_ % MAXC : t_ / VW, hs_ = SEQ ? t_ / MAXC : t_ % VW;
        constexpr int cj = SK_WAVES * jj_ + NW * hs_;
        constexpr int sg = cj >= E2 ? 3 : cj >= E1 ? 2 : cj >= E0 ? 1 : 0;
        constexpr int off = cj - (sg == 3 ? E2 : sg == 2 ? E1 : sg == 1 ? E0 : 0);
        const __amdgpu_buffer_rsrc_t rs = sg == 3 ? rs_a3 : sg == 2 ? rs_a2 : sg == 1 ? rs_a1 : rs_a0;
#pragma unroll
        for (int r = 0; r < RT; ++r) a[j][r] = __builtin_bit_cast(float4, __builtin_amdgcn_raw_buffer_load_b128(rs, ao[sg][r], off * 1024, 0));
        if constexpr (LAY::SUM1 && sg == 1) {
#pragma unroll
            for (int r = 0; r < RT; ++r) a2[SEQ ? hs_ * (LAY::n1 / SK_WAVES) + jj_ - E0 / SK_WAVES : j - FS1][r] = __builtin_bit_cast(float4, __builtin_amdgcn_raw_buffer_load_b128(rs_s1, ao[1][r], off * 1024, 0));
        }
        if constexpr (X3) {
            if constexpr (jj_ % 2 == 0) {
                constexpr int ip = jj_ / 2, hs = hs_;
#pragma unroll
                for (int i = 0; i < CT; ++i)
#pragma unroll
                    for (int pl = 0; pl < 3; ++pl)
                        w3[SEQ ? hs * NPI + ip : ip * VW + hs][i][pl] = __builtin_bit_cast(uint4, __builtin_amdgcn_raw_buffer_load_b128(rs_w3, wo3[i], ((hs * NW * NPI + ip) * 3 + pl) * 1024, 0));
            }
        } else {
#pragma unroll
            for (int i = 0; i < CT; ++i) w[j][i] = __builtin_bit_cast(float4, __builtin_amdgcn_raw_buffer_load_b128(rs_w, wo[i], cj * 1024, 0));
        }
// ... 118 lines not shown
    });
    if constexpr (TIMED) { asm volatile("s_nop 0" :: "v"(acc[0][0][0][0]), "v"(acc[NT - 1][1][VA - 1][0])); }
    L2S_STAMP(4);
    {
        const int col = lane & 15, rb = 4 * (lane >> 4);
#pragma unroll
        for (int h = 0; h < VA; ++h)
#pragma unroll
            for (int q = 0; q < NT; ++q)
#pragma unroll
                for (int r = 0; r < 4; ++r) red[sk_red_idx((wave + NW * (SEQ ? VW - 1 : h)) * NT + q, rb + r, col)] = acc[q][0][h][r] + acc[q][1][h][r];
    }
    __syncthreads();
    L2S_STAMP(5);
    if constexpr (!IS_LSTM) {
#pragma unroll
        for (int n = 0; n < NQ; ++n) {
            const int q = half + NH * n;
            if (q >= NT) continue;
            const int t = tp * CT + q % CT, rt = mg * RT + q / CT;
            if (t >= ntiles || rt >= mts) continue;
            float v = 0.f;
#pragma unroll
            for (int wv = 0; wv < SK_WAVES; ++wv) v += red[sk_red_idx(wv * NT + q, e_row, e_col)];
            v += pf_bias[n];
            const int b = rt * 16 + e_row, np = t * 16 + e_col;
            if (b >= nB) continue;
            if (epi == SK_MEL) {
                if (np < 80) {
                    p.mel[(int64_t)b * p.ld_mel_b + np] = v;
                    if (p.yfrag) p.yfrag[frag16_index(b, np, 80)] = v;
                } else if (np == 80) {
                    p.stop[(int64_t)b * p.ld_stop_b] = v + p.stop_const[b];
                    sk_note_stop(p, b, v + p.stop_const[b]);
                }
                continue;
            }
            if (np >= N) continue;
            v = act_apply(v, act, p.actw, np);
            v += pf_add[n] + pf_row[n];
            if (epi == SK_FRAG) p.out[frag16_index(b, np, p.ldo)] = v;
            else p.out[(int64_t)b * p.ldo + np] = v;
        }
        return;
    }
    L2S_STAMP(6);
#pragma unroll
    for (int cr = 0; cr < NCR; ++cr) {
        if (!cell_on[cr]) continue;
        const int q2 = (tid >> 6) + NW * cr;
        const int t2 = tp * CT + q2 % CT, rt2 = mg * RT + q2 / CT;
        const int b2 = rt2 * 16 + (t64 >> 2), unit2 = t2 * 4 + (t64 & 3);
        const int r2 = t64 >> 2, u2 = t64 & 3;
        float g4[4];
#pragma unroll
        for (int g = 0; g < 4; ++g) {
            float v = 0.f;
#pragma unroll
            for (int wv = 0; wv < SK_WAVES; ++wv) v += red[sk_red_idx(wv * NT + q2, r2, 4 * u2 + g)];
            v += pf_gb[cr][g];
            v += pf_gp[cr][g];
            g4[g] = v;
        }
        const float gi = g4[0], gf = g4[1], gg = g4[2], go = g4[3];
        const float cn = sigmoidf_(gf) * pf_c[cr] + sigmoidf_(gi) * tanhf(gg);
        const float hn = sigmoidf_(go) * tanhf(cn);
        p.c_out[frag16_index(b2, unit2, H)] = cn;
        p.h_out[frag16_index(b2, p.h_out_off + unit2, p.h_out_K)] = hn;
        if (p.h_seq) p.h_seq[(int64_t)b2 * p.ld_hseq + unit2] = hn;
        if (p.h_plain) p.h_plain[(int64_t)b2 * p.ld_hplain + unit2] = hn;
        if constexpr (TRAIN) {
            if (tr->gates) {
                float* gs = tr->gates + (int64_t)b2 * tr->ld_gates + unit2;
                gs[0] = sigmoidf_(gi); gs[H] = sigmoidf_(gf); gs[2 * H] = tanhf(gg); gs[3 * H] = sigmoidf_(go);
            }
            if (tr->c_new) tr->c_new[(int64_t)b2 * tr->ld_c + unit2] = cn;
            if (tr->h_drop) tr->h_drop[frag16_index(b2, unit2, tr->h_drop_K)] = tr->h_mask ? hn * tr->h_mask[(int64_t)b2 * tr->ld_hmask + unit2] : hn;
        }
    }
    if constexpr (TIMED) { asm volatile("s_waitcnt vmcnt(0)" ::: "memory"); }
    L2S_STAMP(7);
}

constexpr int SKP_LO_FLOATS = 2 * 32 * 256, SKP_RING_U4 = 2 * 4 * 12 * 64, SKP_LDS_BYTES = SKP_LO_FLOATS * 4 + SKP_RING_U4 * 16;
static_assert(SKP_LDS_BYTES <= 160 * 1024 && SKP_RING_U4 * 16 >= SKP_LO_FLOATS * 4, "one block per CU; the second half of the partial tiles fits over the ring");
template <class LAY, int DW = 2>
__device__ __forceinline__ void skinny_block_sp(const SkinnyP& p, int tp, int mg, float* lds, int ntiles, int mts) {
    static_assert(LAY::STATIC && LAY::NC % (2 * SK_WAVES) == 0, "static layout, whole chunk pairs per slice");
    constexpr int RT = 4, CT = 2, NW = 4, NT = RT * CT, HR = 2;
    constexpr int MAXC = LAY::NC / SK_WAVES, NPI = MAXC / 2, NST = 2 * NPI;
    constexpr int E0 = LAY::n0, E1 = E0 + LAY::n1, E2 = E1 + LAY::n2;
    const float* const W = p.W;
    const float* const sa0 = p.seg[0].a; const float* const sa1 = p.seg[1].a; const float* const sa2 = p.seg[2].a; const float* const sa3 = p.seg[3].a;
    L2S_PIN_S("s"(W), "s"(sa0), "s"(sa1), "s"(sa2), "s"(sa3), "s"(ntiles), "s"(mts));
    if (tp * 2 * CT >= ntiles) return;
    const int tid = threadIdx.x, lane = tid & 63;
    const int wv8 = __builtin_amdgcn_readfirstlane(tid >> 6);
    const int hc = wv8 >> 2, wave = wv8 & 3;
    const int tph = tp * 2 + hc;
    const __amdgpu_buffer_rsrc_t rs_a0 = __builtin_amdgcn_make_buffer_rsrc(const_cast<float*>(sa0), 0, 0x7fffffff, 0x00020000);
    const __amdgpu_buffer_rsrc_t rs_a1 = __builtin_amdgcn_make_buffer_rsrc(const_cast<float*>(sa1), 0, 0x7fffffff, 0x00020000);
    const __amdgpu_buffer_rsrc_t rs_a2 = __builtin_amdgcn_make_buffer_rsrc(const_cast<float*>(sa2), 0, 0x7fffffff, 0x00020000);
    const __amdgpu_buffer_rsrc_t rs_a3 = __builtin_amdgcn_make_buffer_rsrc(const_cast<float*>(sa3), 0, 0x7fffffff, 0x00020000);
    const __amdgpu_buffer_rsrc_t rs_s1 = __builtin_amdgcn_make_buffer_rsrc(const_cast<float*>(LAY::SUM1 ? p.a_sum : W), 0, 0x7fffffff, 0x00020000);
    const __amdgpu_buffer_rsrc_t rs_w3 = __builtin_amdgcn_make_buffer_rsrc(const_cast<void*>(p.W3), 0, 0x7fffffff, 0x00020000);
    int wo3[CT];
#pragma unroll
    for (int i = 0; i < CT; ++i) wo3[i] = (((min(tph * CT + i, ntiles - 1) * SK_WAVES + wave) * NPI * 3) * 64 + lane) * 16;
    int ao[4][HR];
#pragma unroll
    for (int r = 0; r < HR; ++r) {
        const int rt = min(mg * RT + HR * hc + r, mts - 1);
        ao[0][r] = ((rt * LAY::n0 + wave) * 64 + lane) * 16;
        ao[1][r] = ((rt * LAY::n1 + wave) * 64 + lane) * 16;
        ao[2][r] = ((rt * LAY::n2 + wave) * 64 + lane) * 16;
        ao[3][r] = ((rt * LAY::n3 + wave) * 64 + lane) * 16;
    }
    uint4* const ring = reinterpret_cast<uint4*>(lds + SKP_LO_FLOATS);
    uint4* const ring_rd = ring + wave * 12 * 64 + lane;
    uint4* const ring_wr = ring_rd + HR * hc * 3 * 64;
    float4 a[NST][2][HR], a2[NST][2][HR];
    uint4 w3[NST][CT][3];
    auto load_a = [&](auto sc) {
        constexpr int st = decltype(sc)::value, hs = st / NPI, ip = st % NPI;
#pragma unroll
        for (int c = 0; c < 2; ++c) {
            const int cj = SK_WAVES * (2 * ip + c) + NW * hs;
            const int sg = cj >= E2 ? 3 : cj >= E1 ? 2 : cj >= E0 ? 1 : 0;
            const int off = cj - (sg == 3 ? E2 : sg == 2 ? E1 : sg == 1 ? E0 : 0);
            const __amdgpu_buffer_rsrc_t rs = sg == 3 ? rs_a3 : sg == 2 ? rs_a2 : sg == 1 ? rs_a1 : rs_a0;
#pragma unroll
            for (int r = 0; r < HR; ++r) a[st][c][r] = __builtin_bit_cast(float4, __builtin_amdgcn_raw_buffer_load_b128(rs, ao[sg][r], off * 1024, 0));
            if (LAY::SUM1 && sg == 1) {
#pragma unroll
                for (int r = 0; r < HR; ++r) a2[st][c][r] = __builtin_bit_cast(float4, __builtin_amdgcn_raw_buffer_load_b128(rs_s1, ao[1][r], off * 1024, 0));
            }
        }
    };
    auto load_w = [&](auto sc) {
        constexpr int st = decltype(sc)::value, hs = st / NPI, ip = st % NPI;
#pragma unroll
        for (int i = 0; i < CT; ++i)
#pragma unroll
            for (int pl = 0; pl < 3; ++pl)
                w3[st][i][pl] = __builtin_bit_cast(uint4, __builtin_amdgcn_raw_buffer_load_b128(rs_w3, wo3[i], ((hs * NW * NPI + ip) * 3 + pl) * 1024, 0));
    };
    auto publish = [&](auto sc) {
        constexpr int st = decltype(sc)::value, hs = st / NPI, ip = st % NPI;
#pragma unroll
        for (int c = 0; c < 2; ++c) {
            const int cj = SK_WAVES * (2 * ip + c) + NW * hs;
            if (LAY::SUM1 && cj >= E0 && cj < E1) {
#pragma unroll
                for (int r = 0; r < HR; ++r) {
                    a[st][c][r].x += a2[st][c][r].x; a[st][c][r].y += a2[st][c][r].y; a[st][c][r].z += a2[st][c][r].z; a[st][c][r].w += a2[st][c][r].w;
                }
            }
        }
#pragma unroll
        for (int r = 0; r < HR; ++r) {
            skx_bf16x8 h, m, l;
            skx_split8(a[st][0][r], a[st][1][r], h, m, l);
            uint4* const o = ring_wr + (st & 1) * 4 * 12 * 64 + r * 3 * 64;
            o[0] = __builtin_bit_cast(uint4, h); o[64] = __builtin_bit_cast(uint4, m); o[128] = __builtin_bit_cast(uint4, l);
        }
    };
    __builtin_amdgcn_sched_barrier(0);
    load_a(std::integral_constant<int, 0>{});
    load_w(std::integral_constant<int, 0>{});
    if constexpr (NST > 1) load_a(std::integral_constant<int, 1>{});
    static_for<1, (DW < NST ? DW : NST)>([&](auto sc) { load_w(sc); });
    __builtin_amdgcn_sched_barrier(0);

    const int nB = p.B, H = p.H;
    const float* const bias = p.bias; const float* const pre = p.pre; const int64_t ld_pre = p.ld_pre; const float* const c_in = p.c_in;
    L2S_PIN_S("s"(nB), "s"(H), "s"(bias), "s"(pre), "s"(ld_pre), "s"(c_in));
    const float* const bias_p = bias ? bias : W;
    const float* const add_p = pre ? pre : W;
    constexpr int NCR = NT / NW;
    const int t64 = tid & 63;
    float pf_c[NCR], pf_gb[NCR][4], pf_gp[NCR][4];
    bool cell_on[NCR];
#pragma unroll
    for (int cr = 0; cr < NCR; ++cr) {
        const int q2 = wave + NW * cr;
        const int t2 = tph * CT + q2 % CT, rt2 = mg * RT + q2 / CT;
        const int b2 = rt2 * 16 + (t64 >> 2);
        cell_on[cr] = t2 < ntiles && rt2 < mts && b2 < nB;
        const int t2c = min(t2, ntiles - 1), rt2c = min(rt2, mts - 1);
        const int b2c = min(rt2c * 16 + (t64 >> 2), nB - 1), u2 = t64 & 3;
        pf_c[cr] = c_in[frag16_index(b2c, t2c * 4 + u2, H)];
        const float4 b4 = *reinterpret_cast<const float4*>(bias_p + (bias ? t2c * 16 + 4 * u2 : 0));
        pf_gb[cr][0] = bias ? b4.x : 0.f; pf_gb[cr][1] = bias ? b4.y : 0.f; pf_gb[cr][2] = bias ? b4.z : 0.f; pf_gb[cr][3] = bias ? b4.w : 0.f;
#pragma unroll
        for (int g = 0; g < 4; ++g) {
            const float va = add_p[pre ? (int64_t)b2c * ld_pre + g * H + t2c * 4 + u2 : 0];
            pf_gp[cr][g] = pre ? va : 0.f;
        }
    }
    __builtin_amdgcn_sched_barrier(0);
    publish(std::integral_constant<int, 0>{});
    if constexpr (NST > 2) load_a(std::integral_constant<int, 2>{});
    __syncthreads();

    float* const red_lo = lds + hc * 32 * 256;
    float* const red_hi = lds + SKP_LO_FLOATS + hc * 32 * 256;
    f32x4 acc[NT][2];
#pragma unroll
    for (int q = 0; q < NT; ++q) { acc[q][0] = f32x4{0.f, 0.f, 0.f, 0.f}; acc[q][1] = f32x4{0.f, 0.f, 0.f, 0.f}; }
    static_for<0, NST>([&](auto sc) {
        constexpr int st = decltype(sc)::value, ip = st % NPI, px = ip & 1;
        skx_bf16x8 pl[RT][3];
#pragma unroll
        for (int r = 0; r < RT; ++r)
#pragma unroll
            for (int k = 0; k < 3; ++k) pl[r][k] = __builtin_bit_cast(skx_bf16x8, ring_rd[(st & 1) * 4 * 12 * 64 + (r * 3 + k) * 64]);
        if constexpr (st + 1 < NST) {
            publish(std::integral_constant<int, st + 1>{});
            if constexpr (st + 3 < NST) {
                __builtin_amdgcn_sched_barrier(0);
                load_a(std::integral_constant<int, st + 3>{});
                __builtin_amdgcn_sched_barrier(0);
            }
        }
#define L2S_SKP_TERM(A_, PL_)                                                                                                                  \
        _Pragma("unroll") for (int r = 0; r < RT; ++r)                                                                                         \
            _Pragma("unroll") for (int i = 0; i < CT; ++i)                                                                                     \
                acc[r * CT + i][px] = __builtin_amdgcn_mfma_f32_16x16x32_bf16(pl[r][A_], __builtin_bit_cast(skx_bf16x8, w3[st][i][PL_]), acc[r * CT + i][px], 0, 0, 0);
        L2S_SKP_TERM(2, 0) L2S_SKP_TERM(0, 2) L2S_SKP_TERM(1, 1) L2S_SKP_TERM(1, 0) L2S_SKP_TERM(0, 1) L2S_SKP_TERM(0, 0)
#undef L2S_SKP_TERM
        if constexpr (st + DW < NST) {
            __builtin_amdgcn_sched_barrier(0);
            load_w(std::integral_constant<int, st + DW>{});
            __builtin_amdgcn_sched_barrier(0);
        }
        if constexpr (st == NPI - 1) {
            const int col = lane & 15, rb = 4 * (lane >> 4);
#pragma unroll
            for (int q = 0; q < NT; ++q) {
#pragma unroll
                for (int r = 0; r < 4; ++r) red_lo[sk_red_idx(wave * NT + q, rb + r, col)] = acc[q][0][r] + acc[q][1][r];
                acc[q][0] = f32x4{0.f, 0.f, 0.f, 0.f}; acc[q][1] = f32x4{0.f, 0.f, 0.f, 0.f};
            }
        }
        __syncthreads();
    });
    {
        const int col = lane & 15, rb = 4 * (lane >> 4);
#pragma unroll
        for (int q = 0; q < NT; ++q)
#pragma unroll
            for (int r = 0; r < 4; ++r) red_hi[sk_red_idx(wave * NT + q, rb + r, col)] = acc[q][0][r] + acc[q][1][r];
    }
    __syncthreads();
#pragma unroll
    for (int cr = 0; cr < NCR; ++cr) {
        if (!cell_on[cr]) continue;
        const int q2 = wave + NW * cr;
        const int t2 = tph * CT + q2 % CT, rt2 = mg * RT + q2 / CT;
        const int b2 = rt2 * 16 + (t64 >> 2), unit2 = t2 * 4 + (t64 & 3);
        const int r2 = t64 >> 2, u2 = t64 & 3;
        float g4[4];
#pragma unroll
        for (int g = 0; g < 4; ++g) {
            float v = 0.f;
#pragma unroll
            for (int wv = 0; wv < SK_WAVES; ++wv) v += (wv < NW ? red_lo : red_hi)[sk_red_idx((wv & (NW - 1)) * NT + q2, r2, 4 * u2 + g)];
            v += pf_gb[cr][g];
            v += pf_gp[cr][g];
            g4[g] = v;
        }
        const float gi = g4[0], gf = g4[1], gg = g4[2], go = g4[3];
        const float cn = sigmoidf_(gf) * pf_c[cr] + sigmoidf_(gi) * tanhf(gg);
        const float hn = sigmoidf_(go) * tanhf(cn);
        p.c_out[frag16_index(b2, unit2, H)] = cn;
        p.h_out[frag16_index(b2, p.h_out_off + unit2, p.h_out_K)] = hn;
        if (p.h_seq) p.h_seq[(int64_t)b2 * p.ld_hseq + unit2] = hn;
        if (p.h_plain) p.h_plain[(int64_t)b2 * p.ld_hplain + unit2] = hn;
    }
}

__device__ __forceinline__ double wave_sum_d(double x) {
#pragma unroll
    for (int o = 32; o > 0; o >>= 1) x += __shfl_xor(x, o);
    return x;
}
__device__ __forceinline__ float wave_max_f(float x) {
#pragma unroll
    for (int o = 32; o > 0; o >>= 1) x = fmaxf(x, __shfl_xor(x, o));
    return x;
}
__device__ __forceinline__ float wave_sum_f(float x) {
#pragma unroll
    for (int o = 32; o > 0; o >>= 1) x += __shfl_xor(x, o);
    return x;
}

constexpr int ATT_MAXT = 320;
constexpr int ATT_MAXM = 48;
constexpr int ATT_SM_FLOATS = 512 + ATT_MAXT + 16 + 16;
constexpr int ATT_VLDS_FLOATS = 32 * 256;

__device__ __forceinline__ float block_max8(float x, float* scratch) {
    x = wave_max_f(x);
    __syncthreads();
    if ((threadIdx.x & 63) == 0) scratch[threadIdx.x >> 6] = x;
    __syncthreads();
    float m = scratch[0];
#pragma unroll
    for (int i = 1; i < 8; ++i) m = fmaxf(m, scratch[i]);
    return m;
}
__device__ __forceinline__ float block_sum8(float x, float* scratch) {
    x = wave_sum_f(x);
    __syncthreads();
    if ((threadIdx.x & 63) == 0) scratch[threadIdx.x >> 6] = x;
    __syncthreads();
    return ((scratch[0] + scratch[1]) + (scratch[2] + scratch[3])) + ((scratch[4] + scratch[5]) + (scratch[6] + scratch[7]));
}

#define L2S_ATT_STAMP(k) do { if constexpr (TIMED) { if (threadIdx.x == 0) ats[blockIdx.x * 8 + (k)] = wall_clock64(); } } while (0)
template <bool TRAIN = false, bool TIMED = false, bool VLDS = false, bool SKIP0 = false, bool ML = false>
__device__ __forceinline__ void attention_block(const AttnP& p, int b, float* sm, const AttnTrain* tr = nullptr, unsigned long long* ats = nullptr, int len = 0) {
    static_assert(!SKIP0 || VLDS, "the zero-weight skip rides on the buffer-load form of the inference step");
    static_assert(!ML || (!TRAIN && !TIMED), "per-row lengths: the inference step only");
    L2S_ATT_STAMP(0);
    float* qs = sm;
    float* sc = sm + 512;
    float* scratch = sc + ATT_MAXT;
    const int tid = threadIdx.x, lane = tid & 63;
    const int wave = __builtin_amdgcn_readfirstlane(tid >> 6);
    const int T = p.T;
    const int Te = ML ? len : T;
    const int vcols = p.vp ? 256 : 512;
    const float* const pq = p.q; const float* const pk = p.k; const float* const pv = p.vp ? p.vp : p.v; const float* const ptau = p.tau;
    float* const pav = p.av_frag; float* const pattn = p.attn_out;
    const int ldq = p.ldq, logits = p.attn_logits; const int64_t ld_attn = p.ld_attn_b;
    L2S_PIN_S("s"(T), "s"(pq), "s"(pk), "s"(pv), "s"(ptau), "s"(pav), "s"(pattn), "s"(ldq), "s"(logits), "s"(ld_attn), "s"(vcols));
    const float* kb = pk + (int64_t)b * T * 512 + lane * 8;
    const bool vlane = tid < vcols;
    const float* vb = pv + (int64_t)b * T * vcols + (vlane ? tid : 0);
    const float qv = pq[(int64_t)b * ldq + tid];
    const float tau = ptau[0];
    float4 k0[4], k1[4];
    if constexpr (VLDS) {
        const __amdgpu_buffer_rsrc_t rk = __builtin_amdgcn_make_buffer_rsrc(const_cast<float*>(pk + (int64_t)b * T * 512), 0, Te * 2048, 0x00020000);
#pragma unroll
        for (int r = 0; r < 4; ++r) {
            const int so = __builtin_amdgcn_readfirstlane((wave + 8 * r) * 2048);
            k0[r] = __builtin_bit_cast(float4, __builtin_amdgcn_raw_buffer_load_b128(rk, lane * 32, so, 0));
            k1[r] = __builtin_bit_cast(float4, __builtin_amdgcn_raw_buffer_load_b128(rk, lane * 32, so + 16, 0));
        }
    } else {
#pragma unroll
        for (int r = 0; r < 4; ++r) {
            const int t = wave + 8 * r;
            if (t < Te) {
                k0[r] = *reinterpret_cast<const float4*>(kb + (int64_t)t * 512);
                k1[r] = *reinterpret_cast<const float4*>(kb + (int64_t)t * 512 + 4);
            }
        }
// ... 237 lines not shown
```

### lip2speech_amd/native.py

```python
from __future__ import annotations

import collections
import ctypes
import os
import threading
from typing import Dict, Iterable, Optional

import numpy as np
import torch

_HERE = os.path.dirname(os.path.abspath(__file__))
DIAG_LIB_PATH = os.path.join(_HERE, "csrc", "libl2s_diag.so")
LIB_PATH = os.environ.get("L2S_LIB") or os.path.join(_HERE, "csrc", "libl2s_hip.so")
if LIB_PATH == "diag":
    LIB_PATH = DIAG_LIB_PATH

ABI_SYMBOLS = (
    "l2s_abi_version", "l2s_last_error",
    "l2s_model_create", "l2s_model_set_tensor", "l2s_model_finalize", "l2s_model_destroy",
    "l2s_min_T", "l2s_workspace_bytes", "l2s_state_floats", "l2s_state_offset",
    "l2s_mel_frames", "l2s_mel_targets_workspace_bytes", "l2s_mel_targets",
    "l2s_encoder_fwd", "l2s_normalise_pad_frames", "l2s_build_visual", "l2s_decoder_prologue", "l2s_decode_steps", "l2s_postnet",
    "l2s_workspace_bytes_masked", "l2s_masked_bilstm_plan", "l2s_inference_masked", "l2s_forward_eval_masked", "l2s_decoder_prologue_masked", "l2s_decode_steps_masked",
    "l2s_ragged_plan", "l2s_workspace_bytes_ragged", "l2s_inference_ragged",
    "l2s_forward_eval_ragged_plan", "l2s_workspace_bytes_eval_ragged", "l2s_forward_eval_ragged",
    "l2s_output_lengths", "l2s_inference", "l2s_inference_multi", "l2s_workspace_bytes_multi", "l2s_forward_eval", "l2s_forward_eval_multi", "l2s_model_set_option", "l2s_persist_available", "l2s_persist_timeouts", "l2s_set_thread_chains", "l2s_speaker_workspace_bytes", "l2s_speaker_encoder_fwd",
    "l2s_speaker_packed_plan", "l2s_speaker_workspace_bytes_packed", "l2s_speaker_encoder_packed",
    "l2s_face_workspace_bytes", "l2s_face_encoder_fwd",
    "l2s_inverse_mel_workspace_bytes", "l2s_inverse_mel", "l2s_griffin_lim_workspace_bytes", "l2s_griffin_lim", "l2s_estoi_workspace_bytes", "l2s_estoi_workspace_bytes_long", "l2s_estoi",
    "l2s_set_option",
    "l2s_train_scratch_bytes", "l2s_loss", "l2s_grad_norm", "l2s_adamw_amsgrad_step",
    "l2s_train_steps_tape_floats", "l2s_train_steps_weights_floats", "l2s_train_steps_ws_bytes", "l2s_train_steps_pack_weights",
    "l2s_train_steps_fwd", "l2s_train_steps_bwd",
    "l2s_train_set_bn", "l2s_train_refresh_weights", "l2s_train_encoder_tape_floats", "l2s_train_encoder_ws_bytes", "l2s_train_encoder_fwd", "l2s_train_encoder_bwd",
    "l2s_train_prologue_tape_floats", "l2s_train_prologue_ws_bytes", "l2s_train_prologue_fwd", "l2s_train_prologue_bwd",
    "l2s_train_bind", "l2s_train_postnet_tape_floats", "l2s_train_postnet_ws_bytes", "l2s_train_postnet_fwd", "l2s_train_postnet_bwd",
    "l2s_profile_enable", "l2s_profile_reset", "l2s_profile_count", "l2s_profile_get",
)
DIAG_SYMBOLS = (
    "l2s_op_gemm", "l2s_op_conv1d", "l2s_op_gemm_ex", "l2s_op_conv1d_ex", "l2s_op_conv1d_bwd", "l2s_op_frontend", "l2s_op_launch_chain", "l2s_op_launch_chain2", "l2s_op_skinny_timeline", "l2s_op_attn_timeline", "l2s_op_flat_timeline", "l2s_op_pdecode_timeline", "l2s_op_gemm_x3_timeline", "l2s_op_fused_unit_timeline", "l2s_op_lstm_cell_chain", "l2s_op_step_attn_chain", "l2s_op_stamp_log",
    "l2s_op_face_conv2d", "l2s_op_face_taps", "l2s_op_speaker_taps", "l2s_op_speaker_taps_packed", "l2s_op_encoder_taps",
)

DIAG_OPTIONS = frozenset(("overlap_postnet", "fuse_trunk", "fuse_s2", "skinny_static", "skinny_sized", "skinny_split", "skinny_split8", "skinny_rc", "skinny_rc_jb",
                          "skinny_rc_multi", "skinny_flat", "hoist_vproj", "attn_lds", "flat_half", "half_min_mts", "gemm_x3_dma", "flat_xcd", "attn_skip0", "trunk_chain", "frontend_solo"))

ST_K, ST_V, ST_CKEY, ST_CVAL, ST_ECELL, ST_H, ST_C, ST_ENC, ST_STOPC = range(9)

_lib = None
_diag = None
_process_defaults: Dict[str, int] = {}
_vp, _i, _i64, _fp = ctypes.c_void_p, ctypes.c_int, ctypes.c_int64, ctypes.c_void_p


def _load(path: str) -> ctypes.CDLL:
    if not os.path.exists(path):
        raise RuntimeError(
            f"native library not built: {path} is missing. Build it with "
            "`python -c 'import __graft_entry__ as g; g.build()'` or `make -C lip2speech_amd/csrc` "
            "(hipcc --offload-arch=gfx950). There is no CPU fallback for the Lip2Speech hot path.")
    L = ctypes.CDLL(path)
    _bind(L)
    if hasattr(L, "l2s_op_gemm"):
        _bind_diag(L)
    return L


def lib() -> ctypes.CDLL:
    global _lib
    if _lib is None:
        _lib = _load(LIB_PATH)
    return _lib


def diag() -> ctypes.CDLL:
    global _diag
    if _diag is None:
        _diag = lib() if hasattr(lib(), "l2s_op_gemm") else _load(DIAG_LIB_PATH)
        if _diag is not _lib:
            for name, value in _process_defaults.items():
                check(_diag.l2s_set_option(name.encode(), value), _diag)
            _replay_thread_chains(_diag)
    return _diag


def _bind(L: ctypes.CDLL) -> None:
    L.l2s_last_error.restype = ctypes.c_char_p
    L.l2s_abi_version.restype = _i
    L.l2s_model_create.argtypes = [ctypes.POINTER(_vp)]
    L.l2s_model_set_tensor.argtypes = [_vp, ctypes.c_char_p, _vp, _i64]
    L.l2s_model_finalize.argtypes = [_vp, _vp]
    L.l2s_model_destroy.argtypes = [_vp]
    L.l2s_min_T.argtypes = [_i]
    L.l2s_workspace_bytes.argtypes = [_i] * 5
    L.l2s_workspace_bytes.restype = _i64
    L.l2s_state_floats.argtypes = [_i, _i]
    L.l2s_state_floats.restype = _i64
    L.l2s_state_offset.argtypes = [_i, _i, _i]
    L.l2s_state_offset.restype = _i64
    L.l2s_encoder_fwd.argtypes = [_vp, _fp, _i, _i, _i, _i, _fp, _vp, _i64, _vp]
    L.l2s_normalise_pad_frames.argtypes = [_vp, ctypes.POINTER(_i64), ctypes.POINTER(ctypes.c_int32), _i, _i, _i, _i, _fp, _vp]
    L.l2s_build_visual.argtypes = [_fp, _fp, _i, _i, _fp, _vp]
    L.l2s_decoder_prologue.argtypes = [_vp, _fp, _fp, _fp, _i, _i, _fp, _fp, _vp, _i64, _vp]
    L.l2s_decode_steps.argtypes = [_vp, _fp, _i, _i, _i, _fp, _vp, _fp, _fp, _fp, _i, _vp, _i64, _vp]
    L.l2s_postnet.argtypes = [_vp, _fp, _i, _i, _fp, _fp, _vp, _i64, _vp]
    L.l2s_output_lengths.argtypes = [_fp, _i, _i, _vp, _vp]
    L.l2s_speaker_workspace_bytes.argtypes = [_i, _i]
    L.l2s_speaker_workspace_bytes.restype = _i64
    L.l2s_speaker_encoder_fwd.argtypes = [_vp, _fp, _i, _i, _fp, _vp, _i64, _vp]
    L.l2s_face_workspace_bytes.argtypes = [_i, _i, _i]
    L.l2s_face_workspace_bytes.restype = _i64
    L.l2s_face_encoder_fwd.argtypes = [_vp, _fp, _i64, _i, _i, _i, _fp, _fp, _vp, _i64, _vp]
    L.l2s_inference.argtypes = [_vp, _fp, _fp, _fp, _i, _i, _i, _i, _i, _fp, _vp, _fp, _vp, _i64, _vp]
    L.l2s_workspace_bytes_multi.argtypes = [_i] * 6
    L.l2s_workspace_bytes_multi.restype = _i64
    L.l2s_inference_multi.argtypes = [_vp, _i, ctypes.POINTER(_vp), ctypes.POINTER(_vp), ctypes.POINTER(_vp), _i, _i, _i, _i, _i, _fp, _vp, _fp, _vp, _i64, _vp]
    L.l2s_forward_eval.argtypes = [_vp, _fp, _fp, _fp, _i, _i, _i, _i, _i, _fp, _vp, _fp, _fp, _fp, _fp, _fp, _vp, _i64, _vp]
    L.l2s_forward_eval_multi.argtypes = [_vp, _i, ctypes.POINTER(_vp), ctypes.POINTER(_vp), ctypes.POINTER(_vp), ctypes.POINTER(_vp), _vp,
                                         _i, _i, _i, _i, _i, _fp, _fp, _fp, _fp, _fp, _vp, _i64, _vp]
    L.l2s_model_set_option.argtypes = [_vp, ctypes.c_char_p, _i]
    L.l2s_set_option.argtypes = [ctypes.c_char_p, _i]
    L.l2s_train_bind.argtypes = [_vp, ctypes.c_char_p, _fp, _fp]
    L.l2s_train_postnet_tape_floats.argtypes = [_i, _i]
# ... 19 lines not shown
    L.l2s_train_encoder_fwd.argtypes = [_vp, _fp, _i, _i, _i, _i, _fp, _fp, _fp, _fp, _vp]
    L.l2s_train_encoder_bwd.argtypes = [_vp, _fp, _i, _i, _i, _i, _fp, _i, _fp, _vp, _i64, _vp]
    L.l2s_train_prologue_tape_floats.argtypes = [_i, _i]
    L.l2s_train_prologue_tape_floats.restype = _i64
    L.l2s_train_prologue_ws_bytes.argtypes = [_i, _i]
    L.l2s_train_prologue_ws_bytes.restype = _i64
    L.l2s_train_prologue_fwd.argtypes = [_vp, _fp, _fp, _fp, _i, _i, _fp, _fp, _fp, _vp, _i64, _vp]
    L.l2s_train_prologue_bwd.argtypes = [_vp, _fp, _fp, _i, _i, _fp, _fp, _fp, _fp, _fp, _fp, _fp, _fp, _fp, _fp, _fp, _vp, _i64, _vp]
    L.l2s_train_scratch_bytes.restype = _i64
    L.l2s_loss.argtypes = [_fp] * 6 + [_i, _i, _i] + [_fp] * 5 + [_vp, _vp]
    L.l2s_grad_norm.argtypes = [_fp, _i64, _vp, _fp, _vp]
    _f = ctypes.c_float
    L.l2s_adamw_amsgrad_step.argtypes = [_fp] * 5 + [_i64, _f, _f, _f, _f, _f, _i, _fp, _f, _f, _vp]
    L.l2s_inverse_mel_workspace_bytes.argtypes = [_i] * 6
    L.l2s_inverse_mel_workspace_bytes.restype = _i64
    L.l2s_inverse_mel.argtypes = [_fp, _i, _fp, _i, _fp, _i, _i, _i, _i, _i, _i, _fp, _fp, _vp, _vp, _i64, _vp]
    L.l2s_griffin_lim_workspace_bytes.argtypes = [_i, _i]
    L.l2s_griffin_lim_workspace_bytes.restype = _i64
    L.l2s_griffin_lim.argtypes = [_fp, _fp, _i, _i, _i, _i, _i, ctypes.c_float, _fp, _vp, _i64, _vp]
    L.l2s_estoi_workspace_bytes.argtypes = [_i]
    L.l2s_estoi_workspace_bytes.restype = _i64
    L.l2s_estoi.argtypes = [_fp, _fp, _i, _i, _fp, _i, _i, _i, _i, _i, ctypes.POINTER(ctypes.c_int), _fp, _vp, _i64, _vp]
    if hasattr(L, "l2s_estoi_workspace_bytes_long"):
        L.l2s_estoi_workspace_bytes_long.argtypes = [_i, _i]
        L.l2s_estoi_workspace_bytes_long.restype = _i64
    L.l2s_profile_enable.argtypes = [_i]
    L.l2s_profile_get.argtypes = [_i, ctypes.POINTER(ctypes.c_char_p), ctypes.POINTER(_i64), ctypes.POINTER(ctypes.c_double)]
    if hasattr(L, "l2s_inference_masked"):
        _lens = ctypes.POINTER(ctypes.c_int32)
        L.l2s_workspace_bytes_masked.argtypes = [_i] * 5
        L.l2s_workspace_bytes_masked.restype = _i64
        L.l2s_masked_bilstm_plan.argtypes = [_lens, _i, _i, _lens, _lens, ctypes.POINTER(_i), ctypes.POINTER(_i)]
        L.l2s_inference_masked.argtypes = L.l2s_inference.argtypes + [_lens]
        L.l2s_forward_eval_masked.argtypes = L.l2s_forward_eval.argtypes + [_lens]
        L.l2s_decoder_prologue_masked.argtypes = L.l2s_decoder_prologue.argtypes + [_lens]
        L.l2s_decode_steps_masked.argtypes = L.l2s_decode_steps.argtypes + [_lens]
    if hasattr(L, "l2s_inference_ragged"):
        _lens = ctypes.POINTER(ctypes.c_int32)
        L.l2s_ragged_plan.argtypes = [_i, _lens, _lens, _lens, _lens, _lens, ctypes.POINTER(_i), ctypes.POINTER(_i)]
        L.l2s_workspace_bytes_ragged.argtypes = [_i, _lens, _lens, _i, _i, _i]
        L.l2s_workspace_bytes_ragged.restype = _i64
        L.l2s_inference_ragged.argtypes = [_vp, _i, ctypes.POINTER(_vp), ctypes.POINTER(_vp), ctypes.POINTER(_vp), _lens, _lens, _lens, _i, _i, _i, _fp, _vp, _fp,
                                           _vp, _i64, _vp]
    if hasattr(L, "l2s_forward_eval_ragged"):
        _lens, _offs = ctypes.POINTER(ctypes.c_int32), ctypes.POINTER(_i64)
        L.l2s_forward_eval_ragged_plan.argtypes = [_i, _lens, _lens, _lens, _offs, _offs, _offs, _offs, ctypes.POINTER(_i), ctypes.POINTER(_i), ctypes.POINTER(_i)]
        L.l2s_workspace_bytes_eval_ragged.argtypes = [_i, _lens, _lens, _lens, _i, _i]
        L.l2s_workspace_bytes_eval_ragged.restype = _i64
        L.l2s_forward_eval_ragged.argtypes = [_vp, _i, ctypes.POINTER(_vp), ctypes.POINTER(_vp), ctypes.POINTER(_vp), _lens, _lens, _lens, _lens, _i, _i,
                                              _fp, _fp, _fp, _fp, _fp, _vp, _i64, _vp]
    if hasattr(L, "l2s_mel_targets"):
        L.l2s_mel_frames.argtypes = [_i64]
        L.l2s_mel_frames.restype = _i
        L.l2s_mel_targets_workspace_bytes.argtypes = [_i, _i]
        L.l2s_mel_targets_workspace_bytes.restype = _i64
        L.l2s_mel_targets.argtypes = [_fp, ctypes.POINTER(_i64), ctypes.POINTER(_i64), _i, _fp, _i, _i, _i, _i, _i, ctypes.c_float, _i, _i64, _fp, _fp, _fp, _vp,
                                      _vp, _i64, _vp]
    if hasattr(L, "l2s_speaker_encoder_packed"):
        _lens, _ns = ctypes.POINTER(ctypes.c_int32), ctypes.POINTER(_i64)
        L.l2s_speaker_packed_plan.argtypes = [_ns, _i, _lens, _lens, _lens, ctypes.POINTER(_i), ctypes.POINTER(_i64)]
        L.l2s_speaker_workspace_bytes_packed.argtypes = [_ns, _i]
        L.l2s_speaker_workspace_bytes_packed.restype = _i64
        L.l2s_speaker_encoder_packed.argtypes = [_vp, _fp, _ns, _ns, _i, _fp, _vp, _i64, _vp]


def _bind_diag(L: ctypes.CDLL) -> None:
    L.l2s_op_gemm.argtypes = [_fp, _fp, _fp, _fp, _fp, _fp, _i, _i, _i, _i, _vp]
    L.l2s_op_conv1d.argtypes = [_fp, _fp, _fp, _fp, _fp, _fp, _i, _i, _i, _i, _i, _i, _i, _i, _vp]
    L.l2s_op_gemm_ex.argtypes = [_fp, _fp, _fp, _fp, _fp, _fp, _i, _i, _i, _i, _i, _vp]
    L.l2s_op_conv1d_ex.argtypes = [_fp, _fp, _fp, _fp, _fp, _fp, _i, _i, _i, _i, _i, _i, _i, _i, _i, _vp]
    L.l2s_op_conv1d_bwd.argtypes = [_fp, _fp, _fp, _fp, _fp, _i, _i, _i, _i, _i, _i, _i, _vp]
    L.l2s_op_frontend.argtypes = [_vp, _fp, _i, _i, _i, _i, _fp, _vp]
    L.l2s_op_launch_chain.argtypes = [_i, _i, _i, _i, _fp, _fp, _vp]
    L.l2s_op_skinny_timeline.argtypes = [_vp]
    L.l2s_op_attn_timeline.argtypes = [_vp]
    L.l2s_op_flat_timeline.argtypes = [_vp]
    L.l2s_op_pdecode_timeline.argtypes = [_vp, ctypes.c_int]
    L.l2s_op_gemm_x3_timeline.argtypes = [_vp, ctypes.c_int]
    L.l2s_op_fused_unit_timeline.argtypes = [_vp, _i]
    L.l2s_op_launch_chain2.argtypes = [_i, _i, _i, _i, _fp, _fp, _vp, _vp]
    L.l2s_op_step_attn_chain.argtypes = [_vp, _fp, _i, _i, _i, _vp, _i64, _vp]
    L.l2s_op_lstm_cell_chain.argtypes = [_vp, _i, _i, _vp, _i64, _vp, ctypes.POINTER(ctypes.c_double)]
    L.l2s_op_stamp_log.argtypes = [_vp, _i64]
    L.l2s_op_face_conv2d.argtypes = [_fp, _i64, _i, _i, _i, _i, _fp, _fp, _fp, _fp, _i, _fp, _i, _i, _i, _i, _i, _i, _vp]
    L.l2s_op_face_taps.argtypes = [_vp, _fp, _i64, _i, _vp, _fp, _fp, _vp, _i64, _vp]
    L.l2s_op_speaker_taps.argtypes = [_vp, _fp, _i, _i, _vp, _fp, _vp, _i64, _vp]
    L.l2s_op_speaker_taps_packed.argtypes = [_vp, _fp, ctypes.POINTER(_i64), ctypes.POINTER(_i64), _i, _vp, _fp, _vp, _i64, _vp]
    L.l2s_op_encoder_taps.argtypes = [_vp, _fp, _i, _i, _i, _i, _vp, _fp, _vp, _i64, _vp]


def check(rc: int, L: Optional[ctypes.CDLL] = None) -> None:
    if rc != 0:
        raise RuntimeError("libl2s_hip: " + (L or lib()).l2s_last_error().decode("utf-8", "replace"))


def _dcheck(rc: int) -> None:
    check(rc, diag())


def _stream() -> int:
    return torch.cuda.current_stream().cuda_stream


def _ptr(t: Optional[torch.Tensor]) -> Optional[int]:
    if t is None:
        return None
    assert t.is_cuda and t.is_contiguous(), "device-resident contiguous tensors only"
    return t.data_ptr()


def _f32(t: torch.Tensor) -> torch.Tensor:
    if not t.is_cuda:
        raise RuntimeError("the Lip2Speech hot path runs on the GPU: move inputs to cuda (no CPU fallback)")
    return t.detach().to(torch.float32).contiguous()


def min_T(T: int) -> int:
    return int(lib().l2s_min_T(T))


def video_lengths_array(video_lengths, B: int, T: int):
    if isinstance(video_lengths, torch.Tensor):
        if video_lengths.is_floating_point() or video_lengths.is_complex() or video_lengths.dtype == torch.bool:
            raise TypeError(f"video_lengths must hold integers, got {video_lengths.dtype}")
        arr = video_lengths.detach().cpu().numpy()
    else:
        arr = np.asarray(video_lengths)
        if arr.dtype.kind not in "iu":
            raise TypeError(f"video_lengths must hold integers, got {arr.dtype}")
    if arr.shape != (B,):
        raise ValueError(f"video_lengths must have shape ({B},) - one length per clip - got {tuple(arr.shape)}")
    bad = [(b, int(v)) for b, v in enumerate(arr) if v < 7 or v > T]
    if bad:
        raise ValueError(f"video_lengths outside [7, T = {T}]: " + ", ".join(f"clip {b}: {v}" for b, v in bad))
    return (ctypes.c_int32 * B)(*[int(v) for v in arr])


def masked_bilstm_plan(video_lengths, T: int):
    B = len(video_lengths)
    lens = (ctypes.c_int32 * B)(*[int(v) for v in video_lengths])
    cap, rst = (ctypes.c_int32 * B)(), (ctypes.c_int32 * B)()
    nc, nr = _i(), _i()
    check(lib().l2s_masked_bilstm_plan(lens, B, int(T), cap, rst, ctypes.byref(nc), ctypes.byref(nr)))
    return list(cap[:nc.value]), list(rst[:nr.value])


def workspace_bytes_ragged(batch_B, batch_T, H: int = 96, W: int = 96, S: int = 300) -> int:
    G, i32 = len(batch_B), ctypes.c_int32
    need = int(lib().l2s_workspace_bytes_ragged(G, (i32 * G)(*[int(b) for b in batch_B]), (i32 * G)(*[int(t) for t in batch_T]), H, W, S))
    if need < 0:
        check(1)
    return need


MAX_GROUP = 8
MAX_RAGGED_CLIPS = 256


def ragged_plan(batch_B, batch_T, video_lengths):
    G = len(batch_B)
    flat = [int(v) for v in video_lengths] if not (len(video_lengths) and hasattr(video_lengths[0], "__len__")) else [int(v) for b in video_lengths for v in b]
    n = sum(int(b) for b in batch_B)
    if len(flat) != n:
        raise ValueError(f"video_lengths must hold {n} lengths (sum of batch_B), got {len(flat)}")
    i32 = ctypes.c_int32
    f0, p0 = (i32 * (n + 1))(), (i32 * (n + 1))()
# ... 852 lines not shown
```

Baseline: 3.686 million mel-frames/s.

## Pre-split LSTM hidden states into bf16x3 planes in the producing epilogue

The LSTM cell epilogue now writes each new hidden state a second time as three bf16 planes (hi/mid/lo) in the layout the split-precision skinny kernel consumes. The next step's skinny GEMM loads these pre-split operands directly through buffer loads instead of re-splitting fp32 activations inside the main loop, and the load schedule is adjusted around them. The aim is to cut per-step ALU and register work on the serial decode critical path. The cost is extra workspace, extra epilogue stores, and an initial split/memset. The path is gated on several options (lstm_x3>=5, chains_hint, half_min_mts), so it may not be active.

```diff
diff --git a/include/l2s_diag.h b/include/l2s_diag.h
--- a/include/l2s_diag.h
+++ b/include/l2s_diag.h
@@ -40,6 +40,8 @@
 int l2s_op_step_attn_chain(l2s_model* m, float* state, int B, int T, int n_launches, void* ws, int64_t ws_bytes, void* stream);
 int l2s_op_launch_chain2(int kind, int n_launches, int blocks, int n_per_block, const float* in, float* out, void* stream_a, void* stream_b);
 int l2s_op_stamp_log(void* log_dev, int64_t capacity);
+int64_t l2s_op_plane16_index(int row, int k, int K);
+int64_t l2s_op_decode_plane_bytes(int B);
 
 #ifdef __cplusplus
 }
diff --git a/lip2speech_amd/csrc/l2s_api.hip b/lip2speech_amd/csrc/l2s_api.hip
--- a/lip2speech_amd/csrc/l2s_api.hip
+++ b/lip2speech_amd/csrc/l2s_api.hip
@@ -162,7 +162,7 @@
 }
 static int64_t decode_ws_floats(int B) {
     int64_t Bp = pad16(B);
-    return Bp * (512 * 4 + 512 * 2 + 512 + 256 * 4 + 96) + (int64_t)B * (512 + 256 + 256) + 64 * 24 + (B + 2 + 64)  + (B <= 8 ? pdecode_ws_bytes(B) / 4 + 64 : 0);
+    return Bp * (512 * 4 + 512 * 2 + 512 + 256 * 4 + 96) + 4 * (plane16_bytes((int)Bp, 512) / 4)  + (int64_t)B * (512 + 256 + 256) + 64 * 24 + (B + 2 + 64)  + (B <= 8 ? pdecode_ws_bytes(B) / 4 + 64 : 0);
 }
 constexpr int POST_TAPSPLIT_ROWS = 640;
 static int64_t postnet_ws_floats(int B, int S) { return (int64_t)B * S * 512 * ((int64_t)B * S <= POST_TAPSPLIT_ROWS * MAX_GROUP ? 9 : 4) + 64 * 7; }
@@ -535,6 +535,7 @@
 
 struct DecodeBufs {
     float *h0[2], *h1[2], *c0, *c1, *av, *p1, *cc, *uu, *yf, *p2f, *q, *qc, *p2;
+    unsigned short *h0p[2], *h1p[2];
 };
 
 static int decode_launches(l2s_model* m, float* state, int B, int T, int S, const float* teacher, const uint8_t* teacher_mask,
@@ -553,6 +554,9 @@
     d.p1 = bp.f((int64_t)Bp * 256); d.cc = bp.f((int64_t)Bp * 256); d.uu = bp.f((int64_t)Bp * 256); d.p2f = bp.f((int64_t)Bp * 256);
     d.yf = bp.f((int64_t)Bp * 96);
     d.q = bp.f((int64_t)B * 512); d.qc = bp.f((int64_t)B * 256); d.p2 = bp.f((int64_t)B * 256);
+    for (int i = 0; i < 2; ++i) d.h0p[i] = reinterpret_cast<unsigned short*>(bp.f(plane16_bytes(Bp, 512) / 4));
+    for (int i = 0; i < 2; ++i) d.h1p[i] = reinterpret_cast<unsigned short*>(bp.f(plane16_bytes(Bp, 512) / 4));
+    const bool planes = vsum && skinny_presplit_applies(m->opt, B, 128, w.lstm0.W3 != nullptr) && skinny_presplit_applies(m->opt, B, w.lstm1.tiles, w.lstm1.W3 != nullptr);
     EsCtl* const es = early ? reinterpret_cast<EsCtl*>(bp.f(B + 2)) : nullptr;
     L2S_REQUIRE(!bp.overflow, "decode workspace too small");
     L2S_REQUIRE(!early || !teacher, "early stop is for free-running loops");
@@ -566,6 +570,11 @@
     float* zero256[] = {d.p1, d.cc, d.uu, d.p2f};
     for (float* z : zero256) if (launch_fill(z, (int64_t)Bp * 256, 0.f, s)) return 1;
     if (launch_to_frag(w.bos, 0, B, 80, d.yf, 80, 0, 1, s)) return 1;
+    if (planes) {
+        if (launch_split_frag(d.h0[0], Bp, 512, d.h0p[0], s) || launch_split_frag(d.h1[0], Bp, 512, d.h1p[0], s)) return 1;
+        L2S_CHECK_HIP(hipMemsetAsync(d.h0p[1], 0, plane16_bytes(Bp, 512), s));
+        L2S_CHECK_HIP(hipMemsetAsync(d.h1p[1], 0, plane16_bytes(Bp, 512), s));
+    }
 
     auto fc_group = [&](int step, const float* h1buf, bool write_y) {
         SkinnyP a = sk_base(w.fc, B);
@@ -633,7 +642,9 @@
             a.epi = SK_LSTM; a.H = 512; a.c_in = d.c0; a.c_out = d.c0; a.h_out = d.h0[nxt]; a.h_out_K = 512; a.h_out_off = 0;
             sb.p[0] = a; sb.ntiles[0] = 128; sb.count = 1;
             sb.es_end = es_end; sb.es_step = i - S;
-            if (launch_skinny(sb, s, "step_lstm_cell", m->opt)) return 1;
+            SkPlanes pl;
+            pl.seg[2] = d.h0p[cur]; pl.h_out = d.h0p[nxt];
+            if (launch_skinny(sb, s, "step_lstm_cell", m->opt, planes ? &pl : nullptr)) return 1;
         }
         {
             SkinnyBatch sb{};
@@ -642,7 +653,9 @@
             a.epi = SK_LSTM; a.H = 512; a.c_in = d.c1; a.c_out = d.c1; a.h_out = d.h1[nxt]; a.h_out_K = 512; a.h_out_off = 0;
             sb.p[0] = a; sb.ntiles[0] = w.lstm1.tiles; sb.count = 1;
             sb.es_end = es_end; sb.es_step = i - S;
-            if (launch_skinny(sb, s, "step_lstm_cell", m->opt)) return 1;
+            SkPlanes pl;
+            pl.seg[0] = d.h0p[nxt]; pl.seg[1] = d.h1p[cur]; pl.h_out = d.h1p[nxt];
+            if (launch_skinny(sb, s, "step_lstm_cell", m->opt, planes ? &pl : nullptr)) return 1;
         }
         if (!fold || i == S - 1) {
             SkinnyBatch sb{};
@@ -1765,6 +1778,8 @@
 int l2s_op_pdecode_timeline(void* ts_dev, int step) { pdecode_set_timeline((unsigned long long*)ts_dev, step); return 0; }
 int l2s_op_gemm_x3_timeline(void* ts_dev, int block) { gemm_x3_set_timeline((unsigned long long*)ts_dev, block); return 0; }
 int l2s_op_fused_unit_timeline(void* ts_dev, int h) { shuffle_set_timeline((unsigned long long*)ts_dev, h); return 0; }
+int64_t l2s_op_plane16_index(int row, int k, int K) { return plane16_index(row, k, K); }
+int64_t l2s_op_decode_plane_bytes(int B) { return 4 * plane16_bytes(pad16(B), 512); }
 int l2s_op_stamp_log(void* log_dev, int64_t capacity) {
     L2S_REQUIRE(set_stamp_log((unsigned long long*)log_dev, (long long)capacity) == 0, "stamp log: hipMemcpyToSymbol failed");
     return 0;
diff --git a/lip2speech_amd/csrc/l2s_common.h b/lip2speech_amd/csrc/l2s_common.h
--- a/lip2speech_amd/csrc/l2s_common.h
+++ b/lip2speech_amd/csrc/l2s_common.h
@@ -260,6 +260,15 @@
     return ((int64_t)(rt * (K >> 4) + c) * 64 + (g * 16 + i)) * 4 + e;
 }
 
+constexpr int PLANE16_STRIDE = 64 * 8;
+__host__ __device__ inline int64_t plane16_index(int row, int k, int K) {
+    int rt = row >> 4, i = row & 15, c = k >> 4, g = (k >> 2) & 3, e = k & 3;
+    int pair = (c >> 4) * 8 + (c & 7), second = (c >> 3) & 1;
+    return (((int64_t)(rt * (K >> 5) + pair) * 3) * 64 + (g * 16 + i)) * 8 + second * 4 + e;
+}
+inline int64_t plane16_bytes(int rows16, int K) { return (int64_t)rows16 * K * 6; }
+struct SkPlanes { const void* seg[4] = {nullptr, nullptr, nullptr, nullptr}; unsigned short* h_out = nullptr; };
+
 enum SkinnyEpi {
     SK_PLAIN = 0,
     SK_FRAG = 1,
@@ -307,7 +316,9 @@
 constexpr int SKINNY_MAX_GROUP = 4;
 struct SkinnyBatch { SkinnyP p[SKINNY_MAX_GROUP]; int ntiles[SKINNY_MAX_GROUP]; int count; const int* es_end; int es_step; };
 #define L2S_ES_RETURN(arg) do { if ((arg).es_end && (arg).es_step >= *(arg).es_end) return; } while (0)
-int launch_skinny(const SkinnyBatch& b, hipStream_t s, const char* name, const Options& o = Options());
+int launch_skinny(const SkinnyBatch& b, hipStream_t s, const char* name, const Options& o = Options(), const SkPlanes* planes = nullptr);
+bool skinny_presplit_applies(const Options& o, int rows, int ntiles, bool weight_planes);
+int launch_split_frag(const float* frag, int rows16, int K, unsigned short* planes, hipStream_t s);
 int launch_skx_planes(const float* Wf, int ntiles, int K, void* out, hipStream_t s);
 bool skinny_sum_supported(const Options& o);
 void attn_set_timeline(unsigned long long* ts);
diff --git a/lip2speech_amd/csrc/skinny.hip b/lip2speech_amd/csrc/skinny.hip
--- a/lip2speech_amd/csrc/skinny.hip
+++ b/lip2speech_amd/csrc/skinny.hip
@@ -145,6 +145,48 @@
     static const hipError_t attr_es = hipFuncSetAttribute(reinterpret_cast<const void*>(skinny_sp_kernel<LAYID, true>), hipFuncAttributeMaxDynamicSharedMemorySize, SKP_LDS_BYTES);
     L2S_CHECK_HIP(attr_es);
     SK_ES_LAUNCH(bl.es_end, skinny_sp_kernel, (LAYID), dim3(maxt / 4, (mts + 3) / 4, bl.count), dim3(512), SKP_LDS_BYTES, s, bl, mts);
+    L2S_CHECK_HIP(hipGetLastError());
+    return 0;
+}
+#ifndef L2S_SKP_PA2
+#define L2S_SKP_PA2 2
+#endif
+#ifndef L2S_SKP_PA6
+#define L2S_SKP_PA6 2
+#endif
+template <int LAYID, bool ES = false>
+__global__ __launch_bounds__(512, 1) void skinny_spp_kernel(const SkinnyBatch batch, int mts, const SkPlanes planes) {
+    if constexpr (ES) L2S_ES_RETURN(batch);
+    extern __shared__ __attribute__((aligned(16))) float sp_lds[];
+    L2S_BLOCK_STAMP_BEGIN();
+    skinny_block_sp<typename SkLay<LAYID>::T, 2, true, LAYID == 2 ? L2S_SKP_PA2 : L2S_SKP_PA6>(batch.p[0], blockIdx.x, blockIdx.y, sp_lds, batch.ntiles[0], mts, &planes);
+    L2S_BLOCK_STAMP_END(5u, batch.p[0].c_out);
+}
+template <int LAYID>
+static int launch_spp(const SkinnyBatch& bl, int maxt, int mts, hipStream_t s, const SkPlanes& pl) {
+    static const hipError_t attr = hipFuncSetAttribute(reinterpret_cast<const void*>(skinny_spp_kernel<LAYID, false>), hipFuncAttributeMaxDynamicSharedMemorySize, SKP_LDS_BYTES);
+    L2S_CHECK_HIP(attr);
+    static const hipError_t attr_es = hipFuncSetAttribute(reinterpret_cast<const void*>(skinny_spp_kernel<LAYID, true>), hipFuncAttributeMaxDynamicSharedMemorySize, SKP_LDS_BYTES);
+    L2S_CHECK_HIP(attr_es);
+    SK_ES_LAUNCH(bl.es_end, skinny_spp_kernel, (LAYID), dim3(maxt / 4, (mts + 3) / 4, 1), dim3(512), SKP_LDS_BYTES, s, bl, mts, pl);
+    L2S_CHECK_HIP(hipGetLastError());
+    return 0;
+}
+__global__ __launch_bounds__(256) void skx_split_frag_kernel(const float* __restrict__ frag, int64_t total, int K, unsigned short* __restrict__ planes) {
+    for (int64_t f = (int64_t)blockIdx.x * 256 + threadIdx.x; f < total; f += (int64_t)gridDim.x * 256) {
+        const int e = (int)(f & 3), l = (int)((f >> 2) & 63);
+        const int64_t ch = f >> 8;
+        const int c = (int)(ch % (K >> 4)), rt = (int)(ch / (K >> 4));
+        unsigned short hi, mid, lo;
+        skx_split1(frag[f], hi, mid, lo);
+        unsigned short* const q = planes + plane16_index(16 * rt + (l & 15), 16 * c + 4 * (l >> 4) + e, K);
+        q[0] = hi; q[PLANE16_STRIDE] = mid; q[2 * PLANE16_STRIDE] = lo;
+    }
+}
+int launch_split_frag(const float* frag, int rows16, int K, unsigned short* planes, hipStream_t s) {
+    L2S_REQUIRE(frag && planes && rows16 > 0 && rows16 % 16 == 0 && K > 0 && K % 256 == 0, "split_frag: rows padded to 16, K a multiple of 256");
+    const int64_t total = (int64_t)rows16 * K;
+    hipLaunchKernelGGL(skx_split_frag_kernel, dim3((unsigned)std::min<int64_t>((total + 255) / 256, 2048)), dim3(256), 0, s, frag, total, K, planes);
     L2S_CHECK_HIP(hipGetLastError());
     return 0;
 }
@@ -384,7 +426,13 @@
 static bool skinny_shape_known(int shape) { return shape == 0 || shape == 11 || shape == 21 || shape == 22 || shape == 42; }
 bool skinny_sum_supported(const Options& o) { return o.rc_jb == 0 && g_skinny_ts == nullptr && skinny_shape_known(o.rc_shape) && skinny_shape_known(o.rc_shape_multi); }
 
-int launch_skinny(const SkinnyBatch& b, hipStream_t s, const char* name, const Options& o) {
+bool skinny_presplit_applies(const Options& o, int rows, int ntiles, bool weight_planes) {
+    const int mts = (rows + 15) / 16;
+    return o.lstm_x3 >= 5 && weight_planes && o.rc_jb == 0 && o.rc_shape == 0 && chains_hint() >= 2 && g_skinny_ts == nullptr && o.half_min_mts > 0 &&
+           mts >= o.half_min_mts && mts >= 4 && ntiles > 0 && ntiles % 4 == 0;
+}
+
+int launch_skinny(const SkinnyBatch& b, hipStream_t s, const char* name, const Options& o, const SkPlanes* planes) {
     L2S_REQUIRE(b.count >= 1 && b.count <= SKINNY_MAX_GROUP, "skinny group size");
     int maxt = 0, mts = 0;
     for (int i = 0; i < b.count; ++i) {
@@ -429,7 +477,15 @@
     int x3 = (o.rc_jb == 0 && rc_kind == 2 && (rc_lay == 1 || rc_lay == 2 || rc_lay == 6)) ? o.lstm_x3 : 0;
     if (x3 >= 3 && !overlap) x3 = 2;
     for (int i = 0; i < bl.count; ++i) if (!bl.p[i].W3) x3 = 0;
-    if (x3 == 4) {
+    if (planes) {
+        const SkinnyP& p = bl.p[0];
+        bool ok = bl.count == 1 && x3 >= 5 && shape == 42 && (rc_lay == 2 || rc_lay == 6) && skinny_presplit_applies(o, p.B, bl.ntiles[0], p.W3 != nullptr) &&
+                  planes->h_out && p.H == 512 && p.h_out_K == 512 && p.h_out_off == 0 && !p.h_seq && !p.h_plain;
+        ok = ok && (rc_lay == 2 ? planes->seg[0] && planes->seg[1] && !planes->seg[2] && !planes->seg[3] : !planes->seg[0] && !planes->seg[1] && planes->seg[2] && !planes->seg[3]);
+        L2S_REQUIRE(ok, "skinny: plane operands given to a launch outside the pre-split shared-panel form (skinny_presplit_applies)");
+        return rc_lay == 2 ? launch_spp<2>(bl, maxt, mts, s, *planes) : launch_spp<6>(bl, maxt, mts, s, *planes);
+    }
+    if (x3 >= 4) {
         bool sp = shape == 42 && !g_skinny_ts && o.half_min_mts > 0 && mts >= o.half_min_mts && (rc_lay == 2 || rc_lay == 6);
         for (int i = 0; i < bl.count; ++i) sp = sp && bl.ntiles[i] > 0 && bl.ntiles[i] % 4 == 0;
         if (sp) return rc_lay == 2 ? launch_sp<2>(bl, maxt, mts, s) : launch_sp<6>(bl, maxt, mts, s);
diff --git a/lip2speech_amd/csrc/skinny_dev.h b/lip2speech_amd/csrc/skinny_dev.h
--- a/lip2speech_amd/csrc/skinny_dev.h
+++ b/lip2speech_amd/csrc/skinny_dev.h
@@ -478,6 +478,12 @@
     mid = make_uint2(__builtin_amdgcn_perm(m[1], m[0], 0x07060302u), __builtin_amdgcn_perm(m[3], m[2], 0x07060302u));
     lo = make_uint2(__builtin_amdgcn_perm(l[1], l[0], 0x07060302u), __builtin_amdgcn_perm(l[3], l[2], 0x07060302u));
 }
+__device__ __forceinline__ void skx_split1(float x, unsigned short& hi, unsigned short& mid, unsigned short& lo) {
+    const unsigned xb = __float_as_uint(x);
+    const float r1 = x - __uint_as_float(xb & 0xFFFF0000u);
+    const float r2 = r1 - __uint_as_float(__float_as_uint(r1) & 0xFFFF0000u);
+    hi = (unsigned short)(xb >> 16); mid = (unsigned short)(__float_as_uint(r1) >> 16); lo = (unsigned short)(__float_as_uint(r2) >> 16);
+}
 __device__ __forceinline__ void skx_split8(const float4& a, const float4& b, skx_bf16x8& hi, skx_bf16x8& mid, skx_bf16x8& lo) {
     uint2 h0, m0, l0, h1, m1, l1;
     skx_split4(a, h0, m0, l0); skx_split4(b, h1, m1, l1);
@@ -762,11 +768,15 @@
     L2S_STAMP(7);
 }
 
+template <class LAY> constexpr int skp_seg(int c) { return c >= LAY::n0 + LAY::n1 + LAY::n2 ? 3 : c >= LAY::n0 + LAY::n1 ? 2 : c >= LAY::n0 ? 1 : 0; }
+template <class LAY> constexpr int skp_seg_start(int sg) { return sg == 3 ? LAY::n0 + LAY::n1 + LAY::n2 : sg == 2 ? LAY::n0 + LAY::n1 : sg == 1 ? LAY::n0 : 0; }
+template <class LAY> constexpr bool skp_presplit(int c) { return (skp_seg<LAY>(c) == 0 ? LAY::n0 : skp_seg<LAY>(c) == 1 ? LAY::n1 : skp_seg<LAY>(c) == 2 ? LAY::n2 : LAY::n3) == 32; }
 constexpr int SKP_LO_FLOATS = 2 * 32 * 256, SKP_RING_U4 = 2 * 4 * 12 * 64, SKP_LDS_BYTES = SKP_LO_FLOATS * 4 + SKP_RING_U4 * 16;
 static_assert(SKP_LDS_BYTES <= 160 * 1024 && SKP_RING_U4 * 16 >= SKP_LO_FLOATS * 4, "one block per CU; the second half of the partial tiles fits over the ring");
-template <class LAY, int DW = 2>
-__device__ __forceinline__ void skinny_block_sp(const SkinnyP& p, int tp, int mg, float* lds, int ntiles, int mts) {
+template <class LAY, int DW = 2, bool PS = false, int PA = 0>
+__device__ __forceinline__ void skinny_block_sp(const SkinnyP& p, int tp, int mg, float* lds, int ntiles, int mts, const SkPlanes* pl = nullptr) {
     static_assert(LAY::STATIC && LAY::NC % (2 * SK_WAVES) == 0, "static layout, whole chunk pairs per slice");
+    static_assert(!PS || (LAY::n0 % 16 == 0 && LAY::n1 % 16 == 0 && LAY::n2 % 16 == 0 && LAY::n3 % 16 == 0), "pre-split segments: a K step's chunk pair lies in one segment");
     constexpr int RT = 4, CT = 2, NW = 4, NT = RT * CT, HR = 2;
     constexpr int MAXC = LAY::NC / SK_WAVES, NPI = MAXC / 2, NST = 2 * NPI;
     constexpr int E0 = LAY::n0, E1 = E0 + LAY::n1, E2 = E1 + LAY::n2;
@@ -788,9 +798,16 @@
 #pragma unroll
     for (int i = 0; i < CT; ++i) wo3[i] = (((min(tph * CT + i, ntiles - 1) * SK_WAVES + wave) * NPI * 3) * 64 + lane) * 16;
     int ao[4][HR];
+    [[maybe_unused]] int po[HR];
+    [[maybe_unused]] __amdgpu_buffer_rsrc_t rs_p[4];
+    if constexpr (PS) {
+#pragma unroll
+        for (int j = 0; j < 4; ++j) rs_p[j] = __builtin_amdgcn_make_buffer_rsrc(const_cast<void*>(pl->seg[j] ? pl->seg[j] : (const void*)W), 0, 0x7fffffff, 0x00020000);
+    }
 #pragma unroll
     for (int r = 0; r < HR; ++r) {
         const int rt = min(mg * RT + HR * hc + r, mts - 1);
+        if constexpr (PS) po[r] = (((rt * 16 + wave) * 3) * 64 + lane) * 16;
         ao[0][r] = ((rt * LAY::n0 + wave) * 64 + lane) * 16;
         ao[1][r] = ((rt * LAY::n1 + wave) * 64 + lane) * 16;
         ao[2][r] = ((rt * LAY::n2 + wave) * 64 + lane) * 16;
@@ -800,9 +817,19 @@
     uint4* const ring_rd = ring + wave * 12 * 64 + lane;
     uint4* const ring_wr = ring_rd + HR * hc * 3 * 64;
     float4 a[NST][2][HR], a2[NST][2][HR];
+    [[maybe_unused]] uint4 ap[NST][HR][3];
     uint4 w3[NST][CT][3];
     auto load_a = [&](auto sc) {
         constexpr int st = decltype(sc)::value, hs = st / NPI, ip = st % NPI;
+        if constexpr (PS && skp_presplit<LAY>(SK_WAVES * 2 * ip)) {
+            constexpr int sg = skp_seg<LAY>(SK_WAVES * 2 * ip), j = (SK_WAVES * 2 * ip - skp_seg_start<LAY>(sg)) / 16;
+#pragma unroll
+            for (int r = 0; r < HR; ++r)
+#pragma unroll
+                for (int k = 0; k < 3; ++k)
+                    ap[st][r][k] = __builtin_bit_cast(uint4, __builtin_amdgcn_raw_buffer_load_b128(rs_p[sg], po[r], ((8 * j + NW * hs) * 3 + k) * 1024, 0));
+            return;
+        }
 #pragma unroll
         for (int c = 0; c < 2; ++c) {
             const int cj = SK_WAVES * (2 * ip + c) + NW * hs;
@@ -827,6 +854,26 @@
     };
     auto publish = [&](auto sc) {
         constexpr int st = decltype(sc)::value, hs = st / NPI, ip = st % NPI;
+        if constexpr (PS && skp_presplit<LAY>(SK_WAVES * 2 * ip)) {
+#pragma unroll
+            for (int r = 0; r < HR; ++r) {
+                uint4* const o = ring_wr + (st & 1) * 4 * 12 * 64 + r * 3 * 64;
+                o[0] = ap[st][r][0]; o[64] = ap[st][r][1]; o[128] = ap[st][r][2];
+            }
+            return;
+        }
+#ifdef L2S_SKP_TIMING_RAW
+        constexpr int cj0 = SK_WAVES * (2 * ip) + NW * hs, cj1 = cj0 + SK_WAVES;
+        if constexpr (!(LAY::SUM1 && ((cj0 >= E0 && cj0 < E1) || (cj1 >= E0 && cj1 < E1)))) {
+#pragma unroll
+            for (int r = 0; r < HR; ++r) {
+                uint4* const o = ring_wr + (st & 1) * 4 * 12 * 64 + r * 3 * 64;
+                const uint4 u0 = __builtin_bit_cast(uint4, a[st][0][r]), u1 = __builtin_bit_cast(uint4, a[st][1][r]);
+                o[0] = u0; o[64] = u1; o[128] = make_uint4(u0.x, u1.y, u0.z, u1.w);
+            }
+            return;
+        }
+#endif
 #pragma unroll
         for (int c = 0; c < 2; ++c) {
             const int cj = SK_WAVES * (2 * ip + c) + NW * hs;
@@ -846,6 +893,7 @@
         }
     };
     __builtin_amdgcn_sched_barrier(0);
+    auto moved = [](int t) constexpr { return PS && PA != 0 && skp_presplit<LAY>(SK_WAVES * 2 * (t % NPI)); };
     load_a(std::integral_constant<int, 0>{});
     load_w(std::integral_constant<int, 0>{});
     if constexpr (NST > 1) load_a(std::integral_constant<int, 1>{});
@@ -880,7 +928,7 @@
     }
     __builtin_amdgcn_sched_barrier(0);
     publish(std::integral_constant<int, 0>{});
-    if constexpr (NST > 2) load_a(std::integral_constant<int, 2>{});
+    if constexpr (NST > 2 && !(PA == 2 && moved(2))) load_a(std::integral_constant<int, 2>{});
     __syncthreads();
 
     float* const red_lo = lds + hc * 32 * 256;
@@ -897,7 +945,12 @@
             for (int k = 0; k < 3; ++k) pl[r][k] = __builtin_bit_cast(skx_bf16x8, ring_rd[(st & 1) * 4 * 12 * 64 + (r * 3 + k) * 64]);
         if constexpr (st + 1 < NST) {
             publish(std::integral_constant<int, st + 1>{});
-            if constexpr (st + 3 < NST) {
+            if constexpr (PA == 2 && st + 2 < NST && moved(st + 2)) {
+                __builtin_amdgcn_sched_barrier(0);
+                load_a(std::integral_constant<int, st + 2>{});
+                __builtin_amdgcn_sched_barrier(0);
+            }
+            if constexpr (st + 3 < NST && !moved(st + 3)) {
                 __builtin_amdgcn_sched_barrier(0);
                 load_a(std::integral_constant<int, st + 3>{});
                 __builtin_amdgcn_sched_barrier(0);
@@ -914,6 +967,11 @@
             load_w(std::integral_constant<int, st + DW>{});
             __builtin_amdgcn_sched_barrier(0);
         }
+        if constexpr (PA == 1 && st + 3 < NST && moved(st + 3)) {
+            __builtin_amdgcn_sched_barrier(0);
+            load_a(std::integral_constant<int, st + 3>{});
+            __builtin_amdgcn_sched_barrier(0);
+        }
         if constexpr (st == NPI - 1) {
             const int col = lane & 15, rb = 4 * (lane >> 4);
 #pragma unroll
@@ -957,6 +1015,12 @@
         p.h_out[frag16_index(b2, p.h_out_off + unit2, p.h_out_K)] = hn;
         if (p.h_seq) p.h_seq[(int64_t)b2 * p.ld_hseq + unit2] = hn;
         if (p.h_plain) p.h_plain[(int64_t)b2 * p.ld_hplain + unit2] = hn;
+        if constexpr (PS) {
+            unsigned short hi, mid, lo;
+            skx_split1(hn, hi, mid, lo);
+            unsigned short* const q = pl->h_out + plane16_index(b2, unit2, 512);
+            q[0] = hi; q[PLANE16_STRIDE] = mid; q[2 * PLANE16_STRIDE] = lo;
+        }
     }
 }
 
diff --git a/lip2speech_amd/native.py b/lip2speech_amd/native.py
--- a/lip2speech_amd/native.py
+++ b/lip2speech_amd/native.py
@@ -38,7 +38,7 @@
     "l2s_profile_enable", "l2s_profile_reset", "l2s_profile_count", "l2s_profile_get",
 )
 DIAG_SYMBOLS = (
-    "l2s_op_gemm", "l2s_op_conv1d", "l2s_op_gemm_ex", "l2s_op_conv1d_ex", "l2s_op_conv1d_bwd", "l2s_op_frontend", "l2s_op_launch_chain", "l2s_op_launch_chain2", "l2s_op_skinny_timeline", "l2s_op_attn_timeline", "l2s_op_flat_timeline", "l2s_op_pdecode_timeline", "l2s_op_gemm_x3_timeline", "l2s_op_fused_unit_timeline", "l2s_op_lstm_cell_chain", "l2s_op_step_attn_chain", "l2s_op_stamp_log",
+    "l2s_op_gemm", "l2s_op_conv1d", "l2s_op_gemm_ex", "l2s_op_conv1d_ex", "l2s_op_conv1d_bwd", "l2s_op_frontend", "l2s_op_launch_chain", "l2s_op_launch_chain2", "l2s_op_skinny_timeline", "l2s_op_attn_timeline", "l2s_op_flat_timeline", "l2s_op_pdecode_timeline", "l2s_op_gemm_x3_timeline", "l2s_op_fused_unit_timeline", "l2s_op_lstm_cell_chain", "l2s_op_step_attn_chain", "l2s_op_stamp_log", "l2s_op_plane16_index", "l2s_op_decode_plane_bytes",
     "l2s_op_face_conv2d", "l2s_op_face_taps", "l2s_op_speaker_taps", "l2s_op_speaker_taps_packed", "l2s_op_encoder_taps",
 )
 
@@ -224,6 +224,10 @@
     L.l2s_op_step_attn_chain.argtypes = [_vp, _fp, _i, _i, _i, _vp, _i64, _vp]
     L.l2s_op_lstm_cell_chain.argtypes = [_vp, _i, _i, _vp, _i64, _vp, ctypes.POINTER(ctypes.c_double)]
     L.l2s_op_stamp_log.argtypes = [_vp, _i64]
+    L.l2s_op_plane16_index.argtypes = [_i, _i, _i]
+    L.l2s_op_plane16_index.restype = _i64
+    L.l2s_op_decode_plane_bytes.argtypes = [_i]
+    L.l2s_op_decode_plane_bytes.restype = _i64
     L.l2s_op_face_conv2d.argtypes = [_fp, _i64, _i, _i, _i, _i, _fp, _fp, _fp, _fp, _i, _fp, _i, _i, _i, _i, _i, _i, _vp]
     L.l2s_op_face_taps.argtypes = [_vp, _fp, _i64, _i, _vp, _fp, _fp, _vp, _i64, _vp]
     L.l2s_op_speaker_taps.argtypes = [_vp, _fp, _i, _i, _vp, _fp, _vp, _i64, _vp]
```

Result: slower. 3.643 million mel-frames/s (-1.2%).
